# kakaoenterprise/JORLDY

Hardware: AMD Instinct MI355X
Metric: env_steps_per_s (PPO CartPole sync, W=8 workers/GPU, T=128) (higher is better)
Workload: dtype f32

## Files before the change

### jorldy_amd/csrc/jh_collect.hip

```cpp
#include <chrono>

#include "jh_common.h"

struct jh_persist;
int jh_persist_create(jh_pponet* n, jh_persist** out);
void jh_persist_destroy(jh_persist* p);
int jh_persist_begin(jh_persist* p, int W, int T, hipStream_t st, int split = 0);
unsigned jh_persist_publish(jh_persist* p, int W, const float* h_obs);
unsigned jh_persist_seq(const jh_persist* p);
void jh_persist_publish_rows(jh_persist* p, int r0, int r1, const float* h_obs, unsigned tag);
int jh_persist_collect_range(jh_persist* p, int r0, int n_rows, unsigned tag, float* h_heads);
int jh_persist_collect(jh_persist* p, int W, unsigned tag, float* h_heads);
int jh_persist_collect_rows(jh_persist* p, const int* rows, int n_rows, unsigned tag, float* h_heads);
void jh_persist_abort(jh_persist* p);
bool jh_persist_gave_up(const jh_persist* p);
void jh_persist_dump_debug(jh_persist* p, int T);

namespace {
struct Level {
  void* env = nullptr;
  int S = 0;
  std::vector<float> next, obs, rw;
  std::vector<uint8_t> dn;
  std::vector<int64_t> act;
  void init(int rows, int S_) {
    S = S_;
    next.resize((size_t)S * rows); obs.resize((size_t)S * rows); rw.resize(rows); dn.resize(rows); act.resize(rows);
    for (int i = 0; i < rows; ++i) act[i] = i & 1;
  }
};
inline int fork_step(const jh_env_vtbl& vt, Level& dst, const void* src, int n_src) {
  for (int i = 0; i < n_src; ++i) { vt.copy_row(dst.env, 2 * i, src, i); vt.copy_row(dst.env, 2 * i + 1, src, i); }
  int rc = vt.step(dst.env, 0, 2 * n_src, dst.act.data(), dst.next.data(), dst.rw.data(), dst.dn.data());
  if (rc) return rc;
  return vt.obs(dst.env, 0, 2 * n_src, dst.obs.data());
}
inline void copy_level_row(const jh_env_vtbl& vt, Level& d, int di, const Level& s_, int si) {
  vt.copy_row(d.env, di, s_.env, si);
  const size_t S = (size_t)d.S;
  memcpy(&d.next[S * (size_t)di], &s_.next[S * (size_t)si], sizeof(float) * S);
  memcpy(&d.obs[S * (size_t)di], &s_.obs[S * (size_t)si], sizeof(float) * S);
  d.rw[di] = s_.rw[si];
  d.dn[di] = s_.dn[si];
}
}

struct jh_collector {
  jh_ctx* ctx = nullptr;
  jh_pponet* net = nullptr;
  jh_env_vtbl vt{};
  void* env = nullptr;
  jh_store* store = nullptr;
  int W = 0, S = 0, A = 0;
  int no = 0;
  bool cont = false;
  int col_state = 0, col_action = 1, col_reward = 2, col_next = 3, col_done = 4;
  std::vector<float> obs, next_obs, reward, heads, act_f;
  std::vector<int64_t> act_i;
  std::vector<uint8_t> done;
  bool dbg = false, dbg_persist = false;
  double dbg_publish = 0.0, dbg_wait = 0.0;
  long dbg_n = 0;
  jh_persist* persist = nullptr;
  int mode = 1;
  int lookahead = 1;
  bool split = false;
  Level lv[4];
  void *spec = nullptr, *spec2 = nullptr, *spec3 = nullptr;
  float *cap_h0 = nullptr, *cap_h1 = nullptr, *cap_v = nullptr, *cap_nv = nullptr;
  int64_t cap_rows = 0;
  const void* ride_src[2] = {nullptr, nullptr};
  void* ride_dst[2] = {nullptr, nullptr};
  int64_t ride_bytes[2] = {0, 0};
  void* run = nullptr;
  unsigned *gate_h = nullptr, *gate_d = nullptr, gate_seq = 0;
  int prelaunched_T = 0;
  double t_act = 0, t_env = 0, t_total = 0;
  double t_first = 0, t_extra = 0, t_commit = 0;
  int64_t runs = 0;
  int64_t steps = 0;
};

struct RunState;
static void run_state_alloc(jh_collector* c);
static void run_state_free(jh_collector* c);

static int cart_obs(void* e, int32_t r0, int32_t r1, float* o);
static int ctl_obs(void* e, int32_t r0, int32_t r1, float* o);

static int collector_create(jh_ctx* ctx, jh_pponet* net, const jh_env_vtbl* vt, void* env, jh_store* store, const int32_t* cols,
                            jh_collector** out) {
  JH_ARG(ctx && net && vt && env && store && cols && out);
  JH_ARG(vt->obs && vt->step && vt->W > 0 && vt->S > 0 && vt->A > 0);
  const int W = vt->W, S = vt->S, A = vt->A;
  const bool cont = vt->continuous != 0;
  JH_ARG(net->S == S && net->A == A && (net->cont != 0) == cont);
  JH_ARG(W <= net->max_act_rows);
  for (int i = 0; i < 5; ++i) JH_ARG(cols[i] >= 0 && cols[i] < store->n_cols);
  JH_ARG(store->cols[cols[0]].dtype == JH_F32 && store->cols[cols[0]].elems == S);
  if (cont) JH_ARG(store->cols[cols[1]].dtype == JH_F32 && store->cols[cols[1]].elems == A);
  else JH_ARG(store->cols[cols[1]].dtype == JH_I64 && store->cols[cols[1]].elems == 1);
  JH_ARG(store->cols[cols[2]].dtype == JH_F32 && store->cols[cols[2]].elems == 1);
  JH_ARG(store->cols[cols[3]].dtype == JH_F32 && store->cols[cols[3]].elems == S);
  JH_ARG(store->cols[cols[4]].dtype == JH_U8 && store->cols[cols[4]].elems == 1);
  JH_HIP(hipSetDevice(ctx->device));
  jh_collector* c = new jh_collector();
  c->ctx = ctx; c->net = net; c->vt = *vt; c->env = env; c->store = store; c->W = W; c->S = S; c->A = A; c->cont = cont;
  c->col_state = cols[0]; c->col_action = cols[1]; c->col_reward = cols[2]; c->col_next = cols[3]; c->col_done = cols[4];
  c->no = (cont ? 2 * A : A) + 1;
  c->dbg = getenv("JH_COLLECT_DEBUG") != nullptr;
  c->dbg_persist = getenv("JH_PERSIST_DEBUG") != nullptr;
  if (const char* e = getenv("JH_COLLECT_PERSISTENT")) c->mode = atoi(e);
  if (c->mode == 1 && W <= 32 && W * S <= 512) {
    if (jh_persist_create(net, &c->persist) != JH_OK) c->persist = nullptr;
  }
  const bool forkable = vt->fork_alloc && vt->fork_free && vt->copy_row;
  if (c->persist && forkable && !cont && A == 2 && 3 * W <= 32 && 3 * W * S <= 128) {
    const char* e = getenv("JH_COLLECT_LOOKAHEAD");
    c->lookahead = e ? (atoi(e) >= 2 ? 2 : 1) : 2;
    if (c->lookahead == 2) {
      c->spec = vt->fork_alloc(env, 2 * W); c->spec2 = vt->fork_alloc(env, 4 * W); c->spec3 = vt->fork_alloc(env, 8 * W);
      if (!c->spec || !c->spec2 || !c->spec3) c->lookahead = 1;
    }
  }
  {
    const char* e = getenv("JH_COLLECT_SPLIT");
    c->split = c->persist && c->lookahead != 2 && W == 32 && (vt->obs == cart_obs || vt->obs == ctl_obs) && !(e && atoi(e) == 0);
  }
  c->obs.resize((size_t)S * W);
  c->next_obs.resize((size_t)S * W);
  c->act_i.resize(W);
  c->act_f.resize((size_t)A * W);
  c->reward.resize(W);
  c->done.resize(W);
  c->heads.resize((size_t)c->no * W);
  run_state_alloc(c);
  *out = c;
  return JH_OK;
}

static int cart_obs(void* e, int32_t r0, int32_t r1, float* o) { jh_cartpole_obs_rows((const jh_cartpole*)e, r0, r1, o); return JH_OK; }
static int cart_step(void* e, int32_t r0, int32_t r1, const void* a, float* nx, float* rw, uint8_t* dn) {
  jh_cartpole_step_rows((jh_cartpole*)e, r0, r1, (const int64_t*)a, nx, rw, dn);
  return JH_OK;
}
static void* cart_fork_alloc(void*, int32_t rows) {
  jh_cartpole* e = nullptr;
  return jh_cartpole_create(rows, 0, &e) == JH_OK ? e : nullptr;
}
static void cart_fork_free(void* e) { jh_cartpole_destroy((jh_cartpole*)e); }
static void cart_copy_row(void* d_, int32_t di, const void* s_, int32_t si) {
  jh_cartpole* d = (jh_cartpole*)d_;
  const jh_cartpole* s = (const jh_cartpole*)s_;
  memcpy(&d->s[4 * (size_t)di], &s->s[4 * (size_t)si], sizeof(double) * 4);
  d->t[di] = s->t[si];
  d->rng[di] = s->rng[si];
}
static int ctl_obs(void* e, int32_t r0, int32_t r1, float* o) {
  const jh_control* c = (const jh_control*)e;
  if (r0 < 0 || r1 > c->W || r0 >= r1) return jh_fail(JH_ERR_ARG, "jh_control: rows %d..%d of %d", r0, r1, c->W);
  jh_control_obs_rows(c, r0, r1, o);
  return JH_OK;
}
static int ctl_step(void* e, int32_t r0, int32_t r1, const void* a, float* nx, float* rw, uint8_t* dn) {
  jh_control* c = (jh_control*)e;
  if (r0 < 0 || r1 > c->W || r0 >= r1) return jh_fail(JH_ERR_ARG, "jh_control: rows %d..%d of %d", r0, r1, c->W);
  jh_control_step_rows(c, r0, r1, (const float*)a, nx, rw, dn);
  return JH_OK;
}

JH_EXPORT int jh_collector_create(jh_ctx* ctx, jh_pponet* net, jh_cartpole* env, jh_store* store,
                                  const int32_t* cols ,
                                  jh_collector** out) {
  JH_ARG(env != nullptr);
  const jh_env_vtbl vt{env->W, 4, 2, 0, cart_obs, cart_step, cart_fork_alloc, cart_fork_free, cart_copy_row};
  return collector_create(ctx, net, &vt, env, store, cols, out);
}

JH_EXPORT int jh_collector_create_control(jh_ctx* ctx, jh_pponet* net, jh_control* env, jh_store* store, const int32_t* cols,
                                          jh_collector** out) {
  JH_ARG(env != nullptr);
  const jh_env_vtbl vt{env->W, env->S, env->A, 1, ctl_obs, ctl_step, nullptr, nullptr, nullptr};
  return collector_create(ctx, net, &vt, env, store, cols, out);
}

JH_EXPORT int jh_collector_create_env(jh_ctx* ctx, jh_pponet* net, const jh_env_vtbl* vt, void* env, jh_store* store, const int32_t* cols,
                                      jh_collector** out) {
  return collector_create(ctx, net, vt, env, store, cols, out);
}

JH_EXPORT void jh_collector_destroy(jh_collector* c) {
  if (!c) return;
  if (c->persist) {
    (void)hipSetDevice(c->ctx->device);
    (void)hipDeviceSynchronize();
    jh_persist_destroy(c->persist);
  }
  if (c->gate_h) (void)hipHostFree(c->gate_h);
  if (c->spec) c->vt.fork_free(c->spec);
  if (c->spec2) c->vt.fork_free(c->spec2);
  if (c->spec3) c->vt.fork_free(c->spec3);
  run_state_free(c);
  delete c;
}

JH_EXPORT int jh_collector_set_capture(jh_collector* c, float* d_h0, float* d_h1, float* d_value, float* d_next_value, int64_t rows) {
  JH_ARG(c != nullptr);
  if (!d_value) { c->cap_h0 = c->cap_h1 = c->cap_v = c->cap_nv = nullptr; c->cap_rows = 0; return JH_OK; }
  JH_ARG(d_h0 && d_next_value && rows > 0 && (!c->cont || d_h1));
  c->cap_h0 = d_h0; c->cap_h1 = c->cont ? d_h1 : nullptr; c->cap_v = d_value; c->cap_nv = d_next_value; c->cap_rows = rows;
  return JH_OK;
}

JH_EXPORT int jh_collector_set_ride_along(jh_collector* c, int32_t slot, const void* d_src_mapped, void* d_dst, int64_t bytes) {
  JH_ARG(c != nullptr && slot >= 0 && slot < 2 && bytes >= 0 && (bytes == 0 || (d_src_mapped && d_dst)));
  c->ride_src[slot] = d_src_mapped; c->ride_dst[slot] = d_dst; c->ride_bytes[slot] = bytes;
  return JH_OK;
}

static int collector_steps(const jh_collector* c, int T) {
  const int extra = (c->cap_v && c->cap_rows == (int64_t)c->W * T) ? 1 : 0;
  return (c->lookahead == 2 ? (T + 1) / 2 : T) + extra;
}
static int collector_rows(const jh_collector* c) { return c->lookahead == 2 ? 3 * c->W : c->W; }

JH_EXPORT int jh_collector_prelaunch(jh_collector* c, int32_t T, jh_stream stream) {
  JH_ARG(c != nullptr && T > 0);
  if (!c->persist || c->prelaunched_T) return JH_OK;
  const int steps = collector_steps(c, T);
  int rc = jh_persist_begin(c->persist, collector_rows(c), steps, jh_s(stream), c->split);
  if (rc == JH_OK) c->prelaunched_T = steps;
  return rc;
}

struct RunState {
  bool active = false, cap = false, persistent = false, early = false;
  int T = 0, steps = 0;
  int64_t n = 0;
  float *st = nullptr, *ns = nullptr, *rw = nullptr;
  uint8_t* dn = nullptr;
  int64_t* ac_i = nullptr;
  float* ac_f = nullptr;
  jh_pinned_slab* cap_slab = nullptr;
  float *ch0 = nullptr, *ch1 = nullptr, *cv = nullptr, *cnv = nullptr;
  int stall_t = -1, stall_h = -1;
};
static RunState& run_state(jh_collector* c) { return *static_cast<RunState*>(c->run); }
static void run_state_alloc(jh_collector* c) { c->run = new RunState(); }
static void run_state_free(jh_collector* c) { delete static_cast<RunState*>(c->run); c->run = nullptr; }

static int run_commit(jh_collector* c, RunState& r, int rc_in, const unsigned* wait_flag, unsigned wait_val, hipStream_t st) {
  if (rc_in != JH_OK && wait_flag == nullptr) {
    (void)jh_store_stage_abort(c->store, st);
    if (r.cap_slab) (void)jh_ctx_slab_release(c->ctx, r.cap_slab, st);
    r.cap_slab = nullptr;
    for (int q = 0; q < 2; ++q) { c->ride_src[q] = nullptr; c->ride_dst[q] = nullptr; c->ride_bytes[q] = 0; }
    return rc_in;
  }
  const int A = c->A;
  const int64_t n = r.n;
  const void* xs[6]; void* xd[6]; int64_t xb[6]; int k = 0;
  if (r.cap && rc_in == JH_OK) {
    const char* dev0 = (const char*)r.cap_slab->dev;
    auto job = [&](const float* h, float* d, size_t floats) { xs[k] = dev0 + ((const char*)h - (const char*)r.cap_slab->host); xd[k] = d; xb[k] = (int64_t)(sizeof(float) * floats); ++k; };
    job(r.ch0, c->cap_h0, (size_t)n * A);
    if (c->cont) job(r.ch1, c->cap_h1, (size_t)n * A);
    job(r.cv, c->cap_v, (size_t)n);
    job(r.cnv, c->cap_nv, (size_t)n);
  }
  for (int q = 0; q < 2; ++q) {
    if (rc_in == JH_OK && c->ride_bytes[q] > 0) { xs[k] = c->ride_src[q]; xd[k] = c->ride_dst[q]; xb[k] = c->ride_bytes[q]; ++k; }
    c->ride_src[q] = nullptr; c->ride_dst[q] = nullptr; c->ride_bytes[q] = 0;
  }
  const int rc2 = jh_store_stage_commit_gated(c->store, k, xs, xd, xb, wait_flag, wait_val, st);
  if (r.cap_slab) (void)jh_ctx_slab_release(c->ctx, r.cap_slab, st);
  r.cap_slab = nullptr;
  return rc_in ? rc_in : rc2;
}

static int run_prepare(jh_collector* c, int T, hipStream_t st) {
  if (c->gate_h) {
    const unsigned lost = __atomic_load_n(c->gate_h + 1, __ATOMIC_ACQUIRE);
    if (lost) {
      __atomic_store_n(c->gate_h + 1, 0u, __ATOMIC_RELEASE);
      return jh_fail(JH_ERR_STATE, "the commit launch of an earlier run (tag %u) timed out waiting for its release: that rollout never reached the store and the "
                                   "learner behind it ran on stale rows -- the agent's weights are not trustworthy", lost);
    }
  }
  RunState& r = run_state(c);
  const int W = c->W, A = c->A;
  r = RunState();
  r.T = T;
  r.n = (int64_t)W * T;
  r.cap = c->cap_v && c->cap_rows == r.n;
  r.steps = collector_steps(c, T);
  if (const char* e = getenv("JH_COLLECT_TEST_STALL")) (void)sscanf(e, "%d,%d", &r.stall_t, &r.stall_h);
  void* cols[16] = {};
  int rc = jh_store_stage_begin(c->store, r.n, cols);
  if (rc) return rc;
  r.st = (float*)cols[c->col_state];
  r.ns = (float*)cols[c->col_next];
  r.rw = (float*)cols[c->col_reward];
  r.dn = (uint8_t*)cols[c->col_done];
  r.ac_i = (int64_t*)cols[c->col_action];
  r.ac_f = (float*)cols[c->col_action];
  if (r.cap) {
    const size_t fl = (size_t)r.n * A * (c->cont ? 2 : 1) + 2 * (size_t)r.n;
    rc = jh_ctx_slab(c->ctx, sizeof(float) * fl, &r.cap_slab);
    if (rc) { (void)jh_store_stage_commit(c->store, st); return rc; }
    r.ch0 = (float*)r.cap_slab->host;
    r.ch1 = c->cont ? r.ch0 + (size_t)r.n * A : nullptr;
    r.cv = r.ch0 + (size_t)r.n * A * (c->cont ? 2 : 1);
    r.cnv = r.cv + r.n;
  }
  r.persistent = c->persist != nullptr;
  if (r.persistent) {
    const int pre = c->prelaunched_T;
    c->prelaunched_T = 0;
    if (pre != r.steps || jh_persist_gave_up(c->persist)) {
      if (pre && !jh_persist_gave_up(c->persist)) {
        jh_persist_abort(c->persist);
        (void)hipStreamSynchronize(st);
      }
      rc = jh_persist_begin(c->persist, collector_rows(c), r.steps, st, c->split);
      if (rc) r.persistent = false;
    }
  }
  r.active = true;
  return JH_OK;
}

using Clock = std::chrono::steady_clock;
static double secs(Clock::time_point a, Clock::time_point b) { return std::chrono::duration<double>(b - a).count(); }

static void count_act(jh_collector* c, const RunState& r, int t, double dt) {
  c->t_act += dt;
  if (t == r.T) c->t_extra += dt;
  else if (t == 0) c->t_first += dt;
}

static const void* act_of(const jh_collector* c, int w) {
  return c->cont ? (const void*)(c->act_f.data() + (size_t)c->A * w) : (const void*)(c->act_i.data() + w);
}

static void sample_row(jh_collector* c, const float* z, int w, int training) {
  if (c->cont) jh_sample_continuous(c->net, z, w, training, c->act_f.data() + (size_t)w * c->A);
  else c->act_i[w] = jh_sample_discrete(c->net, z, w, training);
}

static void capture_row(const jh_collector* c, const RunState& r, int w, int t, const float* z) {
  if (!r.cap) return;
  const int A = c->A;
  const float v = z[c->no - 1];
  if (t > 0) r.cnv[(size_t)w * r.T + (t - 1)] = v;
  if (t == r.T) return;
  const size_t row = (size_t)w * r.T + t;
  r.cv[row] = v;
  memcpy(r.ch0 + row * A, z, sizeof(float) * A);
  if (c->cont) memcpy(r.ch1 + row * A, z + A, sizeof(float) * A);
}

static void store_row(const jh_collector* c, const RunState& r, int w, int t, const float* s, const float* s_next, const void* a, float rw, uint8_t dn) {
  const int S = c->S, A = c->A;
  const size_t row = (size_t)w * r.T + t;
  memcpy(r.st + S * row, s, sizeof(float) * S);
  memcpy(r.ns + S * row, s_next, sizeof(float) * S);
  if (c->cont) memcpy(r.ac_f + A * row, a, sizeof(float) * A);
  else r.ac_i[row] = *(const int64_t*)a;
  r.rw[row] = rw;
  r.dn[row] = dn;
}

static int step_rows(jh_collector* c, const RunState& r, int w0, int w1, int t) {
  const int rc = c->vt.step(c->env, w0, w1, act_of(c, 0), c->next_obs.data(), c->reward.data(), c->done.data());
  if (rc) return rc;
  const size_t S = (size_t)c->S;
  for (int w = w0; w < w1; ++w) store_row(c, r, w, t, &c->obs[S * w], &c->next_obs[S * w], act_of(c, w), c->reward[w], c->done[w]);
  return JH_OK;
}

static int act_launch(jh_collector* c, int r0, int n, int training, hipStream_t st) {
  const int A = c->A, no = c->no;
  std::vector<float> mu((size_t)n * A), ls((size_t)n * A), v(n);
  const float* obs = c->obs.data() + (size_t)r0 * c->S;
  const int rc = c->cont ? jh_pponet_act_continuous(c->net, n, obs, c->act_f.data() + (size_t)r0 * A, mu.data(), ls.data(), v.data(), training, (jh_stream)st)
                         : jh_pponet_act_discrete(c->net, n, obs, c->act_i.data() + r0, mu.data(), v.data(), training, (jh_stream)st);
  if (rc) return rc;
  for (int k = 0; k < n; ++k) {
    float* z = c->heads.data() + (size_t)(r0 + k) * no;
    memcpy(z, &mu[(size_t)k * A], sizeof(float) * A);
    if (c->cont) memcpy(z + A, &ls[(size_t)k * A], sizeof(float) * A);
    z[no - 1] = v[k];
  }
  return JH_OK;
}

static int env_failed(jh_collector* c, int rc) {
  jh_persist_abort(c->persist);
  return rc;
}

static int kernel_gave_up(jh_collector* c, const RunState& r, int t, hipStream_t st, int* t_done) {
  jh_persist_abort(c->persist);
  if (r.early)
    return jh_fail(JH_ERR_STATE, "the persistent acting kernel gave up at step %d of a run whose commit was enqueued ahead (jh_collector_begin): "
                                 "no observations for ~0.2 s; use jh_collector_run for environments that may stall", t);
  JH_HIP(hipStreamSynchronize(st));
  *t_done = t;
  return JH_OK;
}


static int run_loop_exchange(jh_collector* c, int training, hipStream_t st, int* t_done) {
  RunState& r = run_state(c);
  const int W = c->W, T = r.T, steps = T + (r.cap ? 1 : 0);
  for (int t = 0; t < steps; ++t) {
    const bool extra = t == T;
    int rc = c->vt.obs(c->env, 0, W, c->obs.data());
    if (rc) return env_failed(c, rc);
    const auto t0 = Clock::now();
    const unsigned tag = jh_persist_publish(c->persist, W, c->obs.data());
    const auto tp = c->dbg ? Clock::now() : t0;
    rc = jh_persist_collect(c->persist, W, tag, c->heads.data());
    if (c->dbg) {
      c->dbg_publish += secs(t0, tp);
      c->dbg_wait += secs(tp, Clock::now());
      c->dbg_n += 1;
    }
    if (rc) return kernel_gave_up(c, r, t, st, t_done);
    for (int w = 0; w < W; ++w) {
      const float* z = c->heads.data() + (size_t)w * c->no;
      if (!extra) sample_row(c, z, w, training);
      capture_row(c, r, w, t, z);
    }
    if (!extra) c->net->act_ctr += 1;
    const auto t1 = Clock::now();
    count_act(c, r, t, secs(t0, t1));
    if (extra) break;
    rc = step_rows(c, r, 0, W, t);
    if (rc) return env_failed(c, rc);
    c->t_env += secs(t1, Clock::now());
    c->steps += 1;
  }
  *t_done = steps;
  if (c->dbg_persist && (c->runs % 16) == 15) jh_persist_dump_debug(c->persist, T);
  if (c->dbg_n > 0 && (c->runs % 4) == 3) {
    fprintf(stderr, "[jh_collect] one timestep per exchange, per step: publish %.2f us, wait + read of the heads %.2f us (sampling + bookkeeping + env step: the rest of act / env)\n",
            c->dbg_publish / c->dbg_n * 1e6, c->dbg_wait / c->dbg_n * 1e6);
    c->dbg_publish = c->dbg_wait = 0.0;
    c->dbg_n = 0;
  }
  return JH_OK;
}

static int run_loop_split(jh_collector* c, int training, hipStream_t st, int* t_done) {
  RunState& r = run_state(c);
  const int W = c->W, T = r.T, steps = T + (r.cap ? 1 : 0), HR = 16;
  const unsigned base = jh_persist_seq(c->persist);
  bool dead = false;
  int rc = c->vt.obs(c->env, 0, W, c->obs.data());
  if (rc) return env_failed(c, rc);
  for (int h = 0; h < 2; ++h) jh_persist_publish_rows(c->persist, h * HR, (h + 1) * HR, c->obs.data(), base + 1);
  for (int t = 0; t < steps; ++t) {
    const bool extra = t == T;
    for (int h = 0; h < 2; ++h) {
      const int r0 = h * HR, r1 = r0 + HR;
      const auto t0 = Clock::now();
      if (t == r.stall_t && h == r.stall_h) {
        while (secs(t0, Clock::now()) < 0.35) {}
      }
      rc = jh_persist_collect_range(c->persist, r0, HR, base + (unsigned)t + 1, c->heads.data() + (size_t)r0 * c->no);
      if (rc) {
        rc = kernel_gave_up(c, r, t, st, t_done);
        if (rc || h == 0) return rc;
        const uint64_t ctr = c->net->act_ctr;
        rc = act_launch(c, r0, HR, 0, st);
        if (rc) return rc;
        c->net->act_ctr = ctr;
        dead = true;
      }
      for (int w = r0; w < r1; ++w) {
        const float* z = c->heads.data() + (size_t)w * c->no;
        if (!extra) sample_row(c, z, w, training);
        capture_row(c, r, w, t, z);
      }
      if (h == 1 && !extra) c->net->act_ctr += 1;
      const auto t1 = Clock::now();
      count_act(c, r, t, secs(t0, t1));
      if (extra) continue;
      rc = step_rows(c, r, r0, r1, t);
      if (rc) return env_failed(c, rc);
      if (t + 1 < steps && !dead) {
        rc = c->vt.obs(c->env, r0, r1, c->obs.data());
        if (rc) return env_failed(c, rc);
        jh_persist_publish_rows(c->persist, r0, r1, c->obs.data(), base + (unsigned)t + 2);
      }
      c->t_env += secs(t1, Clock::now());
    }
    if (!extra) c->steps += 1;
    if (dead) {
      *t_done = t + 1;
      return JH_OK;
    }
  }
  *t_done = steps;
  return JH_OK;
}

static int run_loop_lookahead(jh_collector* c, int training, hipStream_t st, int* t_done) {
  RunState& r = run_state(c);
  const int W = c->W, S = c->S, T = r.T, steps = T + (r.cap ? 1 : 0), no = c->no;
  void* e = c->env;
  const jh_env_vtbl& vt = c->vt;
  Level &L1 = c->lv[0], &L2 = c->lv[1], &L3 = c->lv[2], &tmp = c->lv[3];
  L1.env = c->spec; L2.env = c->spec2; L3.env = c->spec3;
  L1.init(2 * W, S); L2.init(4 * W, S); L3.init(8 * W, S);
  std::vector<float> pub((size_t)3 * W * S), pub_next((size_t)3 * W * S), hz((size_t)W * no), hz2((size_t)W * no);
  std::vector<int> pick(W);
  std::vector<int64_t> a0(W), a1(W);
  int t = 0;
  const bool dbg = c->dbg;
  double d_fork = 0, d_wait = 0, d_sample = 0, d_publish = 0, d_book = 0;
  int n_ex = 0;
  int rc = fork_step(vt, L1, e, W);
  if (!rc) rc = vt.obs(e, 0, W, pub.data());
  if (rc) return env_failed(c, rc);
  memcpy(pub.data() + (size_t)W * S, L1.obs.data(), sizeof(float) * (size_t)2 * W * S);
  auto t0 = Clock::now();
  unsigned tag = jh_persist_publish(c->persist, 3 * W, pub.data());
  while (t < steps) {
    const bool extra = t == T;
    const bool two = !extra && t + 1 < T;
    const int t_next = t + (two ? 2 : 1);
    const auto q0 = dbg ? Clock::now() : Clock::time_point();
    if (!extra) {
      rc = fork_step(vt, L2, L1.env, 2 * W);
      if (!rc && two && t_next < steps) rc = fork_step(vt, L3, L2.env, 4 * W);
      if (rc) return env_failed(c, rc);
    }
    const auto q1 = dbg ? Clock::now() : q0;
    rc = jh_persist_collect_rows(c->persist, nullptr, W, tag, hz.data());
    const auto q2 = dbg ? Clock::now() : q0;
    if (rc) return kernel_gave_up(c, r, t, st, t_done);
    if (!extra) {
      for (int w = 0; w < W; ++w) {
        a0[w] = jh_sample_discrete(c->net, hz.data() + (size_t)w * no, w, training);
        pick[w] = W + 2 * w + (int)a0[w];
      }
      c->net->act_ctr += 1;
      if (two) {
        rc = jh_persist_collect_rows(c->persist, pick.data(), W, tag, hz2.data());
        if (rc) return rc;
        for (int w = 0; w < W; ++w) a1[w] = jh_sample_discrete(c->net, hz2.data() + (size_t)w * no, w, training);
        c->net->act_ctr += 1;
      }
    }
    const auto t1 = Clock::now();
    if (dbg) { d_fork += secs(q0, q1); d_wait += secs(q1, q2); d_sample += secs(q2, t1); ++n_ex; }
    unsigned tag_next = 0;
    auto t0_next = t1;
    if (!extra && t_next < steps) {
      for (int w = 0; w < W; ++w) {
        const int k1 = 2 * w + (int)a0[w];
        if (two) {
          const int k2 = 2 * k1 + (int)a1[w];
          memcpy(&pub_next[(size_t)S * w], &L2.obs[(size_t)S * k2], sizeof(float) * S);
          memcpy(&pub_next[(size_t)S * (W + 2 * w)], &L3.obs[(size_t)S * 2 * k2], sizeof(float) * 2 * S);
        } else {
          memcpy(&pub_next[(size_t)S * w], &L1.obs[(size_t)S * k1], sizeof(float) * S);
          memcpy(&pub_next[(size_t)S * (W + 2 * w)], &L2.obs[(size_t)S * 2 * k1], sizeof(float) * 2 * S);
        }
      }
      t0_next = Clock::now();
      tag_next = jh_persist_publish(c->persist, 3 * W, pub_next.data());
    }
    const auto q3 = dbg ? Clock::now() : t1;
    if (dbg) d_publish += secs(t1, q3);
    for (int w = 0; w < W; ++w) {
      capture_row(c, r, w, t, hz.data() + (size_t)w * no);
      if (two) capture_row(c, r, w, t + 1, hz2.data() + (size_t)w * no);
    }
    count_act(c, r, t, secs(t0, t1));
    if (extra) {
      t = t_next;
      break;
    }
    if (!two) { tmp.env = L3.env; tmp.init(2 * W, S); }
    for (int w = 0; w < W; ++w) {
      const int k1 = 2 * w + (int)a0[w];
      store_row(c, r, w, t, &pub[(size_t)S * w], &L1.next[(size_t)S * k1], &a0[w], L1.rw[k1], L1.dn[k1]);
      if (two) {
        const int k2 = 2 * k1 + (int)a1[w];
        store_row(c, r, w, t + 1, &L1.obs[(size_t)S * k1], &L2.next[(size_t)S * k2], &a1[w], L2.rw[k2], L2.dn[k2]);
        vt.copy_row(e, w, L2.env, k2);
        if (t_next < steps) {
          copy_level_row(vt, L1, 2 * w, L3, 2 * k2);
          copy_level_row(vt, L1, 2 * w + 1, L3, 2 * k2 + 1);
        }
      } else {
        vt.copy_row(e, w, L1.env, k1);
        copy_level_row(vt, tmp, 2 * w, L2, 2 * k1);
        copy_level_row(vt, tmp, 2 * w + 1, L2, 2 * k1 + 1);
      }
    }
    if (!two)
      for (int i = 0; i < 2 * W; ++i) copy_level_row(vt, L1, i, tmp, i);
    c->steps += two ? 2 : 1;
    const auto t2 = Clock::now();
    if (dbg) d_book += secs(q3, t2);
    c->t_env += secs(t1, t2);
    t = t_next;
    tag = tag_next;
    t0 = t0_next;
    pub.swap(pub_next);
  }
  *t_done = t;
  if (dbg && n_ex > 0 && (c->runs % 16) == 15)
    fprintf(stderr, "[jh_collect] host us per exchange (%d exchanges): fork %.2f  wait %.2f  sample %.2f  publish %.2f  book %.2f\n", n_ex, d_fork / n_ex * 1e6,
            d_wait / n_ex * 1e6, d_sample / n_ex * 1e6, d_publish / n_ex * 1e6, d_book / n_ex * 1e6);
  if (c->dbg_persist && (c->runs % 16) == 15) jh_persist_dump_debug(c->persist, collector_steps(c, T));
  return JH_OK;
}

static int run_loop_per_launch(jh_collector* c, int training, hipStream_t st, int t_begin) {
  RunState& r = run_state(c);
  if (r.early) return jh_fail(JH_ERR_STATE, "jh_collector_begin needs the persistent acting kernel (W <= 32, W * S <= 512, JH_COLLECT_PERSISTENT != 0)");
  const int W = c->W, T = r.T, steps = T + (r.cap ? 1 : 0);
  for (int t = t_begin; t < steps; ++t) {
    const bool extra = t == T;
    int rc = c->vt.obs(c->env, 0, W, c->obs.data());
    if (rc) return rc;
    const auto t0 = Clock::now();
    rc = act_launch(c, 0, W, training, st);
    if (rc) return rc;
    if (extra) c->net->act_ctr -= 1;
    for (int w = 0; w < W; ++w) capture_row(c, r, w, t, c->heads.data() + (size_t)w * c->no);
    const auto t1 = Clock::now();
    count_act(c, r, t, secs(t0, t1));
    if (extra) break;
    rc = step_rows(c, r, 0, W, t);
    if (rc) return rc;
    c->t_env += secs(t1, Clock::now());
    c->steps += 1;
  }
  return JH_OK;
}

static int run_loop(jh_collector* c, int training, hipStream_t st) {
  RunState& r = run_state(c);
  int t = 0;
  if (r.persistent) {
    const int rc = c->lookahead == 2 ? run_loop_lookahead(c, training, st, &t)
                   : c->split        ? run_loop_split(c, training, st, &t)
                                     : run_loop_exchange(c, training, st, &t);
    if (rc) return rc;
  }
  return t < r.T + (r.cap ? 1 : 0) ? run_loop_per_launch(c, training, st, t) : JH_OK;
}

JH_EXPORT int jh_collector_run(jh_collector* c, int32_t T, int32_t training, jh_stream stream) {
  JH_ARG(c != nullptr && T > 0);
  if (run_state(c).active) return jh_fail(JH_ERR_STATE, "jh_collector_run inside a jh_collector_begin / jh_collector_loop pair");
  int rc = run_prepare(c, T, jh_s(stream));
  if (rc) return rc;
  rc = run_loop(c, training, jh_s(stream));
  const auto tc = std::chrono::steady_clock::now();
  rc = run_commit(c, run_state(c), rc, nullptr, 0, jh_s(stream));
  c->t_commit += std::chrono::duration<double>(std::chrono::steady_clock::now() - tc).count();
  c->runs += 1;
  run_state(c).active = false;
  return rc;
}

JH_EXPORT int jh_collector_begin(jh_collector* c, int32_t T, jh_stream stream) {
  JH_ARG(c != nullptr && T > 0);
  if (run_state(c).active) return jh_fail(JH_ERR_STATE, "jh_collector_begin twice without jh_collector_loop");
  if (!c->persist) return jh_fail(JH_ERR_STATE, "jh_collector_begin needs the persistent acting kernel (W <= 32, W * S <= 512, JH_COLLECT_PERSISTENT != 0)");
  if (!c->gate_h) {
    JH_HIP(hipHostMalloc((void**)&c->gate_h, 64, hipHostMallocMapped));
    JH_HIP(hipHostGetDevicePointer((void**)&c->gate_d, c->gate_h, 0));
    c->gate_h[0] = 0;
    c->gate_h[1] = 0;
  }
  int rc = run_prepare(c, T, jh_s(stream));
  if (rc) return rc;
  RunState& r = run_state(c);
  if (!r.persistent || !jh_store_commit_is_one_launch(c->store, r.n)) {
    r.early = false;
    return JH_OK;
  }
  r.early = true;
  c->gate_seq = (c->gate_seq + 1) & 0x7fffffffu;
  if (c->gate_seq == 0) c->gate_seq = 1;
  const auto tc = std::chrono::steady_clock::now();
  rc = run_commit(c, r, JH_OK, c->gate_d, c->gate_seq, jh_s(stream));
  c->t_commit += std::chrono::duration<double>(std::chrono::steady_clock::now() - tc).count();
  if (rc) {
    __atomic_store_n(c->gate_h, c->gate_seq, __ATOMIC_RELEASE);
    r.active = false;
  }
  return rc;
}

JH_EXPORT int jh_collector_loop(jh_collector* c, int32_t training, jh_stream stream) {
  JH_ARG(c != nullptr);
  RunState& r = run_state(c);
  if (!r.active) return jh_fail(JH_ERR_STATE, "jh_collector_loop without jh_collector_begin");
  int rc = run_loop(c, training, jh_s(stream));
  if (r.early) {
    __atomic_store_n(c->gate_h, rc == JH_OK ? c->gate_seq : (c->gate_seq | 0x80000000u), __ATOMIC_RELEASE);
  } else {
    const auto tc = std::chrono::steady_clock::now();
    rc = run_commit(c, r, rc, nullptr, 0, jh_s(stream));
    c->t_commit += std::chrono::duration<double>(std::chrono::steady_clock::now() - tc).count();
  }
  c->runs += 1;
  r.active = false;
  return rc;
}

JH_EXPORT int jh_collector_stats_detail(jh_collector* c, double* out6) {
  JH_ARG(c && out6);
  const double r = c->runs > 0 ? (double)c->runs : 1.0;
  out6[0] = c->t_first / r * 1e6;
  out6[1] = c->t_extra / r * 1e6;
  out6[2] = c->t_commit / r * 1e6;
  const double inner = (double)c->steps - (double)c->runs;
  out6[3] = inner > 0 ? (c->t_act - c->t_first - c->t_extra) / inner * 1e6 : 0.0;
  out6[4] = (double)c->runs;
  out6[5] = (double)c->steps;
  return JH_OK;
}

JH_EXPORT int jh_collector_stats(jh_collector* c, double* act_us_per_step, double* env_us_per_step, int32_t reset) {
  JH_ARG(c != nullptr);
  const double n = c->steps > 0 ? (double)c->steps : 1.0;
  if (act_us_per_step) *act_us_per_step = c->t_act / n * 1e6;
  if (env_us_per_step) *env_us_per_step = c->t_env / n * 1e6;
  if (reset) { c->t_act = c->t_env = c->t_first = c->t_extra = c->t_commit = 0; c->steps = 0; c->runs = 0; }
  return JH_OK;
}
```

### jorldy_amd/csrc/jh_persist.hip

```cpp
#if defined(__x86_64__)
#include <emmintrin.h>
#endif

#include "jh_common.h"

typedef float f32x4 __attribute__((ext_vector_type(4)));

struct PersistArgs {
  int W, S, H, n_out, T, G;
  const float *W1, *b1, *W2, *b2;
  const float* wh[12];
  const float* hbias[12];
  const unsigned long long* obs_gran;
  float4* part;
  int rows_ld;
  unsigned* abort_flag;
  unsigned seq0;
  long max_polls;
  unsigned long long* dbg;
  int period;
  unsigned long long* mbox;
  float4* dpart;
  int split;
};

__device__ __forceinline__ void persist_poll_issue(const void* gsrc, unsigned lds_off) {
  unsigned keep;
  asm volatile("s_mov_b32 %0, m0\n\ts_mov_b32 m0, %2\n\ts_nop 0\n\tglobal_load_lds_dwordx4 %1, off sc0 sc1\n\ts_mov_b32 m0, %0"
               : "=&s"(keep) : "v"(gsrc), "s"(lds_off) : "memory");
}

template <int SP, int NCH, int D, int PI>
__global__ void __launch_bounds__(256, 1) jh_act_persist_kernel(PersistArgs p) {
  constexpr bool W1LDS = SP > 8;
  constexpr int NJ = 2 * PI;
  __shared__ __attribute__((aligned(16))) unsigned long long s_ring[D][128 * PI];
  __shared__ __attribute__((aligned(16))) float s_w1[W1LDS ? 64 * NCH * SP : 4];
  __shared__ __attribute__((aligned(16))) float s_x[2][16][SP];
  __shared__ __attribute__((aligned(16))) float s_acc[2][4][64][4];
  __shared__ float s_h2[16][17];
  __shared__ float s_wh[12][16];
  __shared__ float s_b2[16], s_hb[12];
  __shared__ __attribute__((aligned(16))) float s_out[16][12];
  __shared__ int s_go[2];
  __shared__ __attribute__((aligned(16))) f32x4 s_red[32][64];
  const int H = p.H, S = p.S;
  const int lane = threadIdx.x & 63, wid = __builtin_amdgcn_readfirstlane(threadIdx.x >> 6);
  const int tiles_n = H / 16;
  const int tile = blockIdx.x % tiles_n, rt = blockIdx.x / tiles_n, n0 = tile * 16;
  const int r = lane & 15, kq = lane >> 4;
  const int kbeg = wid * 16 * NCH;
  float w2f[NCH][4], b1f[NCH][4], w1f[NCH][4][W1LDS ? 1 : SP];
#pragma unroll
  for (int u = 0; u < NCH; ++u) {
    const int kb = kbeg + 16 * u + 4 * kq;
#pragma unroll
    for (int j = 0; j < 4; ++j) {
      w2f[u][j] = p.W2[(size_t)(n0 + r) * H + kb + j];
      b1f[u][j] = p.b1[kb + j];
      if (!W1LDS) {
#pragma unroll
        for (int q = 0; q < SP; ++q) w1f[u][j][q] = q < S ? p.W1[(size_t)(kb + j) * S + q] : 0.f;
      }
    }
  }
  if (W1LDS) {
    for (int i = threadIdx.x; i < H * SP; i += 256) {
      const int k = i / SP, q = i - k * SP;
      s_w1[i] = q < S ? p.W1[(size_t)k * S + q] : 0.f;
    }
  }
  for (int i = threadIdx.x; i < 12 * 16; i += 256) {
    const int o = i >> 4, c = i & 15;
    s_wh[o][c] = o < p.n_out ? p.wh[o][n0 + c] : 0.f;
  }
  if (threadIdx.x < 16) s_b2[threadIdx.x] = p.b2[n0 + threadIdx.x];
  if (threadIdx.x < 12) s_hb[threadIdx.x] = threadIdx.x < p.n_out ? *p.hbias[threadIdx.x] : 0.f;
  for (int i = threadIdx.x; i < 2 * 16 * SP; i += 256) (&s_x[0][0][0])[i] = 0.f;
  for (int i = threadIdx.x; i < D * 128 * PI; i += 256) (&s_ring[0][0])[i] = 0ull;
  __syncthreads();

  const int g0 = p.split ? rt * 16 * S : 0;
  const int n_gran = p.split ? (p.W - 16 * rt < 16 ? p.W - 16 * rt : 16) * S : p.W * S;
  const int n16 = (n_gran + 1) >> 1;
  const char* my_src = reinterpret_cast<const char*>(p.obs_gran + g0) + 16 * (lane < n16 ? lane : 0);
  const bool poller = !p.mbox || (p.split ? tile == 0 : blockIdx.x == 0);
  unsigned long long next_issue = 0;
  int slot = 0;
  const unsigned ring_lane = (unsigned)(uintptr_t)&s_ring[0][0] + 8u * (unsigned)lane;
  __builtin_amdgcn_s_waitcnt(0x0F70);
  if (wid == 0 && poller) {
#pragma unroll
    for (int d = 0; d < D; ++d) {
#pragma unroll
      for (int q = 0; q < PI; ++q)
        if (64 * q + lane < n16) persist_poll_issue(my_src + 1024 * q, __builtin_amdgcn_readfirstlane((unsigned)(uintptr_t)&s_ring[d][0]) + 1024u * q);
    }
    next_issue = wall_clock64();
  }

  for (int t = 1; t <= p.T; ++t) {
    const int par = t & 1;
    const unsigned tag = p.seq0 + (unsigned)t;
    if (wid == 0 && !poller) {
      bool ok = false;
      for (long spin = 0; spin < p.max_polls * 4; ++spin) {
        unsigned long long gq[NJ];
        bool mine = true;
#pragma unroll
        for (int j = 0; j < NJ; ++j) {
          const int g = 64 * j + lane;
          gq[j] = (j == 0 || 64 * j < n_gran) ? __hip_atomic_load(p.mbox + g0 + (g < n_gran ? g : 0), __ATOMIC_RELAXED, __HIP_MEMORY_SCOPE_AGENT) : 0ull;
          mine = mine && (g >= n_gran || (unsigned)(gq[j] >> 32) == tag);
        }
        if (__all(mine)) {
#pragma unroll
          for (int j = 0; j < NJ; ++j) {
            const int g = 64 * j + lane, gg = g0 + g;
            if (g < n_gran && (gg / S) >> 4 == rt) s_x[par][(gg / S) & 15][gg % S] = __uint_as_float((unsigned)gq[j]);
          }
          ok = true;
          break;
        }
        if ((spin & 1023) == 1023 && __hip_atomic_load(p.abort_flag, __ATOMIC_RELAXED, __HIP_MEMORY_SCOPE_SYSTEM) != 0) break;
      }
      if (lane == 0) s_go[par] = ok ? 1 : 0;
    } else if (wid == 0) {
      bool ok = false;
      for (long spin = 0; spin < p.max_polls; ++spin) {
        asm volatile("s_waitcnt vmcnt(%0)" ::"n"(PI * (D - 1)) : "memory");
        unsigned long long gq[NJ];
        {
          const unsigned ra = ring_lane + (unsigned)slot * (1024u * PI);
          if constexpr (PI == 1) {
            asm volatile("ds_read_b64 %0, %2\n\tds_read_b64 %1, %2 offset:512\n\ts_waitcnt lgkmcnt(0)" : "=&v"(gq[0]), "=&v"(gq[1]) : "v"(ra) : "memory");
          } else if constexpr (PI == 2) {
            asm volatile("ds_read_b64 %0, %4\n\tds_read_b64 %1, %4 offset:512\n\tds_read_b64 %2, %4 offset:1024\n\tds_read_b64 %3, %4 offset:1536\n\ts_waitcnt lgkmcnt(0)"
                         : "=&v"(gq[0]), "=&v"(gq[1]), "=&v"(gq[2]), "=&v"(gq[3]) : "v"(ra) : "memory");
          } else if constexpr (PI == 3) {
            asm volatile("ds_read_b64 %0, %6\n\tds_read_b64 %1, %6 offset:512\n\tds_read_b64 %2, %6 offset:1024\n\tds_read_b64 %3, %6 offset:1536\n\t"
                         "ds_read_b64 %4, %6 offset:2048\n\tds_read_b64 %5, %6 offset:2560\n\ts_waitcnt lgkmcnt(0)"
                         : "=&v"(gq[0]), "=&v"(gq[1]), "=&v"(gq[2]), "=&v"(gq[3]), "=&v"(gq[4]), "=&v"(gq[5]) : "v"(ra) : "memory");
          } else {
            static_assert(PI == 4, "1 .. 4 poll instructions per poll are spelled out");
            asm volatile("ds_read_b64 %0, %8\n\tds_read_b64 %1, %8 offset:512\n\tds_read_b64 %2, %8 offset:1024\n\tds_read_b64 %3, %8 offset:1536\n\t"
                         "ds_read_b64 %4, %8 offset:2048\n\tds_read_b64 %5, %8 offset:2560\n\tds_read_b64 %6, %8 offset:3072\n\tds_read_b64 %7, %8 offset:3584\n\ts_waitcnt lgkmcnt(0)"
                         : "=&v"(gq[0]), "=&v"(gq[1]), "=&v"(gq[2]), "=&v"(gq[3]), "=&v"(gq[4]), "=&v"(gq[5]), "=&v"(gq[6]), "=&v"(gq[7]) : "v"(ra) : "memory");
          }
        }
        bool mine = true;
#pragma unroll
        for (int j = 0; j < NJ; ++j) mine = mine && (64 * j + lane >= n_gran || (unsigned)(gq[j] >> 32) == tag);
        const bool done = __all(mine);
        if (done) {
#pragma unroll
          for (int j = 0; j < NJ; ++j) {
            const int g = 64 * j + lane, gg = g0 + g;
            if (g < n_gran) {
              if ((gg / S) >> 4 == rt) s_x[par][(gg / S) & 15][gg % S] = __uint_as_float((unsigned)gq[j]);
              if (p.mbox) __hip_atomic_store(p.mbox + gg, gq[j], __ATOMIC_RELAXED, __HIP_MEMORY_SCOPE_AGENT);
            }
          }
        }
        if (p.period > 0 && !done) {
          while (wall_clock64() < next_issue) __builtin_amdgcn_s_sleep(1);
        }
        next_issue = wall_clock64() + (unsigned long long)p.period;
#pragma unroll
        for (int q = 0; q < PI; ++q)
          if (64 * q + lane < n16) persist_poll_issue(my_src + 1024 * q, __builtin_amdgcn_readfirstlane((unsigned)(uintptr_t)&s_ring[slot][0]) + 1024u * q);
        slot = __builtin_amdgcn_readfirstlane(slot + 1 == D ? 0 : slot + 1);
        if (done) { ok = true; break; }
        if ((spin & 255) == 255 && __hip_atomic_load(p.abort_flag, __ATOMIC_RELAXED, __HIP_MEMORY_SCOPE_SYSTEM) != 0) break;
      }
      if (lane == 0) s_go[par] = ok ? 1 : 0;
    }
    __syncthreads();
    if (p.dbg && blockIdx.x == 0 && threadIdx.x == 0) { p.dbg[(t - 1) * 8 + 0] = wall_clock64(); p.dbg[(t - 1) * 8 + 1] = __builtin_readcyclecounter(); }
    if (!s_go[par]) {
      if (threadIdx.x == 0) __hip_atomic_store(p.abort_flag, 2u, __ATOMIC_RELAXED, __HIP_MEMORY_SCOPE_SYSTEM);
      break;
    }
    float xr[SP];
#pragma unroll
    for (int q4 = 0; q4 < SP / 4; ++q4) {
      const float4 v = *reinterpret_cast<const float4*>(&s_x[par][r][4 * q4]);
      xr[4 * q4] = v.x; xr[4 * q4 + 1] = v.y; xr[4 * q4 + 2] = v.z; xr[4 * q4 + 3] = v.w;
    }
    f32x4 acc = (f32x4){0.f, 0.f, 0.f, 0.f}, acc2 = (f32x4){0.f, 0.f, 0.f, 0.f};
#pragma unroll
    for (int u = 0; u < NCH; ++u) {
#pragma unroll
      for (int j = 0; j < 4; ++j) {
        float a = 0.f;
        if (W1LDS) {
          const float* wr = s_w1 + (size_t)(kbeg + 16 * u + 4 * kq + j) * SP;
#pragma unroll
          for (int q4 = 0; q4 < SP / 4; ++q4) {
            const float4 w = *reinterpret_cast<const float4*>(wr + 4 * q4);
            a = fmaf(xr[4 * q4], w.x, a); a = fmaf(xr[4 * q4 + 1], w.y, a); a = fmaf(xr[4 * q4 + 2], w.z, a); a = fmaf(xr[4 * q4 + 3], w.w, a);
          }
        } else {
#pragma unroll
          for (int q = 0; q < SP; ++q) a = fmaf(xr[q], w1f[u][j][q], a);
        }
        a += b1f[u][j];
        a = a > 0.f ? a : 0.f;
        if (j & 1) acc2 = __builtin_amdgcn_mfma_f32_16x16x4f32(a, w2f[u][j], acc2, 0, 0, 0);
        else acc = __builtin_amdgcn_mfma_f32_16x16x4f32(a, w2f[u][j], acc, 0, 0, 0);
      }
    }
#pragma unroll
    for (int i = 0; i < 4; ++i) s_acc[par][wid][lane][i] = acc[i] + acc2[i];
    __syncthreads();
    if (wid == 0) {
      float hv[4];
#pragma unroll
      for (int i = 0; i < 4; ++i) {
        float v = ((s_acc[par][0][lane][i] + s_acc[par][1][lane][i]) + s_acc[par][2][lane][i]) + s_acc[par][3][lane][i];
        v += s_b2[r];
        hv[i] = v > 0.f ? v : 0.f;
      }
#pragma unroll
      for (int i = 0; i < 4; ++i) s_h2[kq * 4 + i][r] = hv[i];
      __builtin_amdgcn_wave_barrier();
      __builtin_amdgcn_fence(__ATOMIC_RELEASE, "workgroup");
      f32x4 ph = (f32x4){0.f, 0.f, 0.f, 0.f};
#pragma unroll
      for (int c = 0; c < 4; ++c) {
        const float av = s_h2[r][4 * c + kq];
        const float bv = r < 12 ? s_wh[r][4 * c + kq] : 0.f;
        ph = __builtin_amdgcn_mfma_f32_16x16x4f32(av, bv, ph, 0, 0, 0);
      }
      if (r < 12) {
#pragma unroll
        for (int i = 0; i < 4; ++i) s_out[kq * 4 + i][r] = ph[i] + (tile == 0 ? s_hb[r] : 0.f);
      }
      __builtin_amdgcn_wave_barrier();
      __builtin_amdgcn_fence(__ATOMIC_RELEASE, "workgroup");
      const int g = lane >> 4, row = lane & 15;
      if (g < p.G && 16 * rt + row < p.W) {
        const f32x4 gq = (f32x4){s_out[row][3 * g], s_out[row][3 * g + 1], s_out[row][3 * g + 2], __uint_as_float(tag)};
        if (p.dpart) {
          float4* dst = p.dpart + ((size_t)(rt * p.G + g) * 16 + row) * tiles_n + tile;
          asm volatile("global_store_dwordx4 %0, %1, off sc1\n\ts_nop 1" ::"v"(dst), "v"(gq) : "memory");
        } else {
          float4* dst = p.part + ((size_t)tile * p.G + g) * p.rows_ld + 16 * rt + row;
          asm volatile("global_store_dwordx4 %0, %1, off sc0 sc1\n\ts_nop 1" ::"v"(dst), "v"(gq) : "memory");
        }
      }
    }
    if (p.dpart && tile == 0) {
      const int g = lane >> 4, row = lane & 15;
      const bool mine = g < p.G && 16 * rt + row < p.W;
      const int per = tiles_n / 4;
      bool ok = true;
      if (mine) {
        const float4* src = p.dpart + ((size_t)(rt * p.G + g) * 16 + row) * tiles_n + wid * per;
        f32x4 q[8];
        long spin = 0;
        for (;;) {
          const float4* a1 = per > 4 ? src + 4 : src;
          asm volatile("global_load_dwordx4 %0, %8, off sc1\n\tglobal_load_dwordx4 %1, %9, off sc1\n\tglobal_load_dwordx4 %2, %10, off sc1\n\t"
                       "global_load_dwordx4 %3, %11, off sc1\n\tglobal_load_dwordx4 %4, %12, off sc1\n\tglobal_load_dwordx4 %5, %12, off offset:16 sc1\n\t"
                       "global_load_dwordx4 %6, %12, off offset:32 sc1\n\tglobal_load_dwordx4 %7, %12, off offset:48 sc1\n\ts_waitcnt vmcnt(0)"
                       : "=&v"(q[0]), "=&v"(q[1]), "=&v"(q[2]), "=&v"(q[3]), "=&v"(q[4]), "=&v"(q[5]), "=&v"(q[6]), "=&v"(q[7])
                       : "v"(src), "v"(src + (per > 1 ? 1 : 0)), "v"(src + (per > 2 ? 2 : 0)), "v"(src + (per > 2 ? 3 : 0)), "v"(a1)
                       : "memory");
          bool all = true, newer = false;
#pragma unroll
          for (int j = 0; j < 8; ++j) {
            const unsigned seen = __float_as_uint(q[j][3]);
            if (j < per) {
              all = all && seen == tag;
              newer = newer || (int)(seen - tag) > 0;
            }
          }
          if (all) break;
          if (newer || ++spin > 2000000L || ((spin & 1023) == 1023 && __hip_atomic_load(p.abort_flag, __ATOMIC_RELAXED, __HIP_MEMORY_SCOPE_SYSTEM) != 0)) { ok = false; break; }
        }
#pragma unroll
        for (int j = 0; j < 8; ++j)
          if (j < per) s_red[wid * per + j][lane] = ok ? q[j] : (f32x4){0.f, 0.f, 0.f, __uint_as_float(tag + 0x40000000u)};
      }
      __syncthreads();
      if (wid == 1 && mine) {
        float z0 = 0.f, z1 = 0.f, z2 = 0.f;
        bool good = true;
        for (int tt = 0; tt < tiles_n; ++tt) {
          const f32x4 v = s_red[tt][lane];
          good = good && __float_as_uint(v[3]) == tag;
          z0 += v[0]; z1 += v[1]; z2 += v[2];
        }
        if (good) {
          const f32x4 gq = (f32x4){z0, z1, z2, __uint_as_float(tag)};
          float4* dst = p.part + (size_t)g * p.rows_ld + 16 * rt + row;
          asm volatile("global_store_dwordx4 %0, %1, off sc0 sc1\n\ts_nop 1" ::"v"(dst), "v"(gq) : "memory");
        }
      }
    }
    if (p.dbg && blockIdx.x == 0 && threadIdx.x == 0) { p.dbg[(t - 1) * 8 + 4] = wall_clock64(); p.dbg[(t - 1) * 8 + 5] = __builtin_readcyclecounter(); }
  }
  asm volatile("s_waitcnt vmcnt(0)" ::: "memory");
}

constexpr int kPersistMaxGranules = 512;
struct jh_persist {
  jh_pponet* net = nullptr;
  unsigned long long* gran_h = nullptr;
  unsigned long long* gran_d = nullptr;
  float4 *part_h = nullptr, *part_d = nullptr;
  unsigned *flag_h = nullptr, *flag_d = nullptr;
  unsigned seq = 0;
  int tiles = 0, n_out = 0, G = 0;
  int rows_ld = 16;
  unsigned long long *dbg_h = nullptr, *dbg_d = nullptr;
  unsigned long long* mbox = nullptr;
  float4* dpart = nullptr;
  bool reduced = false;
  int rows_published = 0;
  bool split = false;
};

static int persist_heads(const jh_pponet* n) { return (n->cont ? 2 * n->A : n->A) + 1; }

int jh_persist_create(jh_pponet* n, jh_persist** out) {
  JH_ARG(n && out);
  const int H = n->H, S = n->S;
  JH_ARG(S >= 1 && S <= 16 && (H == 64 || H == 128 || H == 256 || H == 512) && persist_heads(n) <= 12);
  jh_persist* p = new jh_persist();
  p->net = n;
  p->tiles = H / 16;
  p->n_out = persist_heads(n);
  p->G = (p->n_out + 2) / 3;
  JH_HIP(hipHostMalloc((void**)&p->gran_h, sizeof(unsigned long long) * kPersistMaxGranules, hipHostMallocMapped));
  JH_HIP(hipHostGetDevicePointer((void**)&p->gran_d, p->gran_h, 0));
  const size_t part_bytes = sizeof(float4) * 32 * (size_t)p->tiles * p->G;
  JH_HIP(hipHostMalloc((void**)&p->part_h, part_bytes, hipHostMallocMapped));
  memset(p->part_h, 0, part_bytes);
  JH_HIP(hipHostGetDevicePointer((void**)&p->part_d, p->part_h, 0));
  JH_HIP(hipHostMalloc((void**)&p->flag_h, sizeof(unsigned) * 16, hipHostMallocMapped));
  JH_HIP(hipHostGetDevicePointer((void**)&p->flag_d, p->flag_h, 0));
  JH_HIP(hipMalloc((void**)&p->mbox, sizeof(unsigned long long) * kPersistMaxGranules));
  JH_HIP(hipMemset(p->mbox, 0, sizeof(unsigned long long) * kPersistMaxGranules));
  JH_HIP(hipMalloc((void**)&p->dpart, sizeof(float4) * (2 * 4 * 16 * (size_t)p->tiles + 8)));
  JH_HIP(hipMemset(p->dpart, 0, sizeof(float4) * (2 * 4 * 16 * (size_t)p->tiles + 8)));
  memset(p->gran_h, 0, sizeof(unsigned long long) * kPersistMaxGranules);
  memset(p->flag_h, 0, sizeof(unsigned) * 16);
  if (getenv("JH_PERSIST_DEBUG")) {
    p->dbg_h = (unsigned long long*)malloc(sizeof(unsigned long long) * 8 * 4096);
    JH_HIP(hipMalloc((void**)&p->dbg_d, sizeof(unsigned long long) * 8 * 4096));
  }
  p->seq = 1000;
  *out = p;
  return JH_OK;
}

void jh_persist_destroy(jh_persist* p) {
  if (!p) return;
  (void)hipHostFree(p->gran_h);
  (void)hipHostFree(p->part_h);
  (void)hipHostFree(p->flag_h);
  (void)hipFree(p->mbox);
  (void)hipFree(p->dpart);
  if (p->dbg_d) (void)hipFree(p->dbg_d);
  free(p->dbg_h);
  delete p;
}

template <int SP, int NCH>
static void persist_launch(int depth, int pi, int grid, hipStream_t st, const PersistArgs& a) {
  if (pi == 2) JH_LAUNCH_NAMED("jh_act_persist_kernel", (jh_act_persist_kernel<SP, NCH, 4, 2>), dim3(grid), dim3(256), 0, st, a);
  else if (pi == 3) JH_LAUNCH_NAMED("jh_act_persist_kernel", (jh_act_persist_kernel<SP, NCH, 4, 3>), dim3(grid), dim3(256), 0, st, a);
  else if (pi == 4) JH_LAUNCH_NAMED("jh_act_persist_kernel", (jh_act_persist_kernel<SP, NCH, 4, 4>), dim3(grid), dim3(256), 0, st, a);
  else if (depth >= 4) JH_LAUNCH_NAMED("jh_act_persist_kernel", (jh_act_persist_kernel<SP, NCH, 4, 1>), dim3(grid), dim3(256), 0, st, a);
  else if (depth >= 2) JH_LAUNCH_NAMED("jh_act_persist_kernel", (jh_act_persist_kernel<SP, NCH, 2, 1>), dim3(grid), dim3(256), 0, st, a);
  else JH_LAUNCH_NAMED("jh_act_persist_kernel", (jh_act_persist_kernel<SP, NCH, 1, 1>), dim3(grid), dim3(256), 0, st, a);
}

int jh_persist_begin(jh_persist* p, int W, int T, hipStream_t st, int split) {
  jh_pponet* n = p->net;
  JH_ARG(W > 0 && W <= 32 && W * n->S <= kPersistMaxGranules && T > 0 && (!split || W == 32));
  const int win = split ? 16 * n->S : W * n->S;
  const int pi = ((win + 1) / 2 + 63) / 64;
  PersistArgs a{};
  a.W = W; a.S = n->S; a.H = n->H; a.T = T; a.G = p->G;
  a.W1 = n->params + n->o_w1; a.b1 = n->params + n->o_b1; a.W2 = n->params + n->o_w2; a.b2 = n->params + n->o_b2;
  int o = 0;
  for (int k = 0; k < n->A; ++k, ++o) { a.wh[o] = n->params + n->o_wh0 + (int64_t)k * n->H; a.hbias[o] = n->params + n->o_bh0 + k; }
  if (n->cont)
    for (int k = 0; k < n->A; ++k, ++o) { a.wh[o] = n->params + n->o_wh1 + (int64_t)k * n->H; a.hbias[o] = n->params + n->o_bh1 + k; }
  a.wh[o] = n->params + n->o_wv; a.hbias[o] = n->params + n->o_bv; ++o;
  a.n_out = o;
  a.obs_gran = p->gran_d; a.part = p->part_d; a.abort_flag = p->flag_d;
  a.seq0 = p->seq;
  a.dbg = p->dbg_d;
  static const int depth = getenv("JH_PERSIST_DEPTH") ? atoi(getenv("JH_PERSIST_DEPTH")) : 4;
  static const int period = getenv("JH_PERSIST_PERIOD") ? atoi(getenv("JH_PERSIST_PERIOD")) : 10;
  a.period = depth > 1 ? period : 0;
  static const int relay = getenv("JH_PERSIST_RELAY") ? atoi(getenv("JH_PERSIST_RELAY")) : 1;
  a.mbox = relay ? p->mbox : nullptr;
  const int reduce = getenv("JH_PERSIST_REDUCE") ? atoi(getenv("JH_PERSIST_REDUCE")) : (split ? 1 : 0);
  p->reduced = reduce == 1;
  a.dpart = p->reduced ? p->dpart : nullptr;
  a.split = split ? 1 : 0;
  p->split = split != 0;
  a.max_polls = 600000;
  p->flag_h[0] = 0;
  const int nch = n->H / 64;
  const int sp = (n->S + 3) / 4 * 4;
  const int rt = W > 16 ? 2 : 1;
  p->rows_ld = 16 * rt;
  a.rows_ld = p->rows_ld;
  const int grid = p->tiles * rt;
#define JH_PERSIST_CASE(NCH)                                   \
  if (nch == NCH) {                                            \
    if (sp == 4) persist_launch<4, NCH>(depth, pi, grid, st, a);   \
    else if (sp == 8) persist_launch<8, NCH>(depth, pi, grid, st, a);   \
    else if (sp == 12) persist_launch<12, NCH>(depth, pi, grid, st, a); \
    else persist_launch<16, NCH>(depth, pi, grid, st, a);          \
  }
  JH_PERSIST_CASE(1) else JH_PERSIST_CASE(2) else JH_PERSIST_CASE(4) else JH_PERSIST_CASE(8)
#undef JH_PERSIST_CASE
  JH_LAUNCH_CHECK();
  return JH_OK;
}

unsigned jh_persist_publish(jh_persist* p, int W, const float* h_obs) {
  const unsigned tag = ++p->seq;
  p->rows_published = W;
  const int n = W * p->net->S;
  for (int i = 0; i < n; ++i) {
    unsigned bits;
    memcpy(&bits, h_obs + i, 4);
    __atomic_store_n(p->gran_h + i, ((unsigned long long)tag << 32) | bits, __ATOMIC_RELEASE);
  }
  return tag;
}

unsigned jh_persist_seq(const jh_persist* p) { return p->seq; }
void jh_persist_publish_rows(jh_persist* p, int r0, int r1, const float* h_obs, unsigned tag) {
  const int S = p->net->S;
  if (r1 > p->rows_published) p->rows_published = r1;
  for (int i = r0 * S; i < r1 * S; ++i) {
    unsigned bits;
    memcpy(&bits, h_obs + i, 4);
    __atomic_store_n(p->gran_h + i, ((unsigned long long)tag << 32) | bits, __ATOMIC_RELEASE);
  }
  if ((int)(tag - p->seq) > 0) p->seq = tag;
}

static int persist_collect(jh_persist* p, const int* rows, int n_rows, unsigned tag, float* h_heads, int r_first, bool block_order);
int jh_persist_collect_rows(jh_persist* p, const int* rows, int n_rows, unsigned tag, float* h_heads) {
  return persist_collect(p, rows, n_rows, tag, h_heads, 0, !rows && n_rows > 16);
}
int jh_persist_collect_range(jh_persist* p, int r0, int n_rows, unsigned tag, float* h_heads) { return persist_collect(p, nullptr, n_rows, tag, h_heads, r0, true); }
static int persist_collect(jh_persist* p, const int* rows, int n_rows, unsigned tag, float* h_heads, int r_first, bool block_order) {
  const int n_out = p->n_out, G = p->G, ld = p->rows_ld, tiles = p->reduced ? 1 : p->tiles;
  volatile unsigned* abort_w = p->flag_h;
  struct alignas(16) Gran16 { unsigned w[4]; };
  const Gran16* part = reinterpret_cast<const Gran16*>(p->part_h);
  float z[32][12];
  unsigned char have[32];
  JH_ARG(n_rows <= 32);
  if (block_order) {
    for (int k = 0; k < n_rows; ++k)
      for (int o = 0; o < 12; ++o) z[k][o] = 0.f;
    long spins = 0;
    for (int t = 0; t < tiles; ++t)
      for (int g = 0; g < G; ++g) {
        const Gran16* blk = part + ((size_t)t * G + g) * ld + r_first;
        for (;;) {
          bool all = true;
          for (int k = 0; k < n_rows; ++k)
            if (__atomic_load_n(reinterpret_cast<const unsigned*>(blk + k) + 3, __ATOMIC_ACQUIRE) != tag) { all = false; break; }
          if (all) break;
          if (++spins >= 40000000L || ((spins & 1023) == 1023 && *abort_w == 2u))
            return jh_fail(JH_ERR_STATE, "persistent acting kernel did not answer step tag %u", tag);
          __builtin_ia32_pause();
        }
        for (int k = 0; k < n_rows; ++k) {
          alignas(16) unsigned w4[4];
#if defined(__x86_64__)
          _mm_store_si128(reinterpret_cast<__m128i*>(w4), _mm_load_si128(reinterpret_cast<const __m128i*>(blk + k)));
#else
          memcpy(w4, blk + k, 16);
#endif
          if (w4[3] != tag) return jh_fail(JH_ERR_STATE, "persistent acting kernel: granule of step tag %u rewritten while it was read", tag);
          float f3[3];
          memcpy(f3, w4, 12);
          z[k][3 * g] += f3[0]; z[k][3 * g + 1] += f3[1]; z[k][3 * g + 2] += f3[2];
        }
      }
    for (int k = 0; k < n_rows; ++k) memcpy(h_heads + (size_t)k * n_out, z[k], sizeof(float) * n_out);
    return JH_OK;
  }
  int missing = n_rows;
  const int pf_rows = (!rows && p->rows_published > n_rows) ? p->rows_published - n_rows : 0;
  for (int k = 0; k < n_rows; ++k) have[k] = 0;
  for (long spin = 0; spin < 40000000L && missing; ++spin) {
    for (int k = 0; k < n_rows; ++k) {
      if (have[k]) continue;
      const int wq = rows ? rows[k] : k;
      float acc[12] = {0, 0, 0, 0, 0, 0, 0, 0, 0, 0, 0, 0};
      bool ok = true;
      for (int t = 0; t < tiles && ok; ++t)
        for (int g = 0; g < G; ++g) {
          const Gran16* gp = part + ((size_t)t * G + g) * ld + wq;
          if (__atomic_load_n(reinterpret_cast<const unsigned*>(gp) + 3, __ATOMIC_ACQUIRE) != tag) { ok = false; break; }
#if defined(__x86_64__)
          if (pf_rows > 0 && k == 0) {
            const char* q = reinterpret_cast<const char*>(part + ((size_t)t * G + g) * ld + n_rows);
            for (int b = 0; b < pf_rows * 16; b += 64) _mm_prefetch(q + b, _MM_HINT_T0);
          }
#endif
          alignas(16) unsigned w4[4];
#if defined(__x86_64__)
          _mm_store_si128(reinterpret_cast<__m128i*>(w4), _mm_load_si128(reinterpret_cast<const __m128i*>(gp)));
#else
          memcpy(w4, gp, 16);
#endif
          if (w4[3] != tag) { ok = false; break; }
          float f3[3];
          memcpy(f3, w4, 12);
          acc[3 * g] += f3[0]; acc[3 * g + 1] += f3[1]; acc[3 * g + 2] += f3[2];
        }
      if (ok) {
        memcpy(z[k], acc, sizeof(acc));
        have[k] = 1;
        --missing;
      }
    }
    if (missing) {
      if ((spin & 1023) == 1023 && *abort_w == 2u) break;
      __builtin_ia32_pause();
    }
  }
  if (missing) return jh_fail(JH_ERR_STATE, "persistent acting kernel did not answer step tag %u", tag);
  for (int k = 0; k < n_rows; ++k) memcpy(h_heads + (size_t)k * n_out, z[k], sizeof(float) * n_out);
  return JH_OK;
}

int jh_persist_collect(jh_persist* p, int W, unsigned tag, float* h_heads) { return jh_persist_collect_rows(p, nullptr, W, tag, h_heads); }

int jh_persist_heads(const jh_persist* p) { return p->n_out; }

void jh_persist_dump_debug(jh_persist* p, int T) {
  if (!p->dbg_h) return;
  (void)hipDeviceSynchronize();
  (void)hipMemcpy(p->dbg_h, p->dbg_d, sizeof(unsigned long long) * 8 * (size_t)T, hipMemcpyDeviceToHost);
  double a = 0, c = 0, cyc = 0;
  for (int t = 1; t < T; ++t) {
    const unsigned long long* d = p->dbg_h + (size_t)t * 8;
    const unsigned long long* pr = p->dbg_h + (size_t)(t - 1) * 8;
    a += (double)(d[0] - pr[4]);
    c += (double)(d[4] - d[0]);
    cyc += (double)(d[5] - d[1]) / ((double)(d[4] - d[0]) + 1e-9);
  }
  const double n = T - 1;
  fprintf(stderr, "[jh_persist] per step (wall_clock64 ticks = 10 ns): wait %.1f  compute %.1f ; shader clock ~%.0f MHz\n",
          a / n, c / n, cyc / n * 100.0);
}

bool jh_persist_gave_up(const jh_persist* p) { return __atomic_load_n(p->flag_h, __ATOMIC_ACQUIRE) == 2u; }

void jh_persist_abort(jh_persist* p) { __atomic_store_n(p->flag_h, 1u, __ATOMIC_RELEASE); }
```

Baseline: 1.220 million.

## Split lookahead exchange into two pipelined halves with variable row counts

```diff
diff --git a/jorldy_amd/csrc/jh_collect.hip b/jorldy_amd/csrc/jh_collect.hip
--- a/jorldy_amd/csrc/jh_collect.hip
+++ b/jorldy_amd/csrc/jh_collect.hip
@@ -5,11 +5,12 @@
 struct jh_persist;
 int jh_persist_create(jh_pponet* n, jh_persist** out);
 void jh_persist_destroy(jh_persist* p);
-int jh_persist_begin(jh_persist* p, int W, int T, hipStream_t st, int split = 0);
+bool jh_persist_can_split(const jh_persist* p, int rows0, int rows1);
+int jh_persist_begin(jh_persist* p, int W, int T, hipStream_t st, const int* half_rows);
 unsigned jh_persist_publish(jh_persist* p, int W, const float* h_obs);
 unsigned jh_persist_seq(const jh_persist* p);
-void jh_persist_publish_rows(jh_persist* p, int r0, int r1, const float* h_obs, unsigned tag);
-int jh_persist_collect_range(jh_persist* p, int r0, int n_rows, unsigned tag, float* h_heads);
+void jh_persist_publish_rows(jh_persist* p, int row0, int n, const float* h_obs, unsigned tag);
+int jh_persist_collect_range(jh_persist* p, int r0, int n_rows, unsigned tag, float* h_heads, int pf_rows);
 int jh_persist_collect(jh_persist* p, int W, unsigned tag, float* h_heads);
 int jh_persist_collect_rows(jh_persist* p, const int* rows, int n_rows, unsigned tag, float* h_heads);
 void jh_persist_abort(jh_persist* p);
@@ -29,11 +30,12 @@
     for (int i = 0; i < rows; ++i) act[i] = i & 1;
   }
 };
-inline int fork_step(const jh_env_vtbl& vt, Level& dst, const void* src, int n_src) {
-  for (int i = 0; i < n_src; ++i) { vt.copy_row(dst.env, 2 * i, src, i); vt.copy_row(dst.env, 2 * i + 1, src, i); }
-  int rc = vt.step(dst.env, 0, 2 * n_src, dst.act.data(), dst.next.data(), dst.rw.data(), dst.dn.data());
+inline int fork_step(const jh_env_vtbl& vt, Level& dst, const void* src, int i0, int i1) {
+  for (int i = i0; i < i1; ++i) { vt.copy_row(dst.env, 2 * i, src, i); vt.copy_row(dst.env, 2 * i + 1, src, i); }
+  const size_t r0 = 2 * (size_t)i0, S = (size_t)dst.S;
+  int rc = vt.step(dst.env, 2 * i0, 2 * i1, dst.act.data() + r0, dst.next.data() + S * r0, dst.rw.data() + r0, dst.dn.data() + r0);
   if (rc) return rc;
-  return vt.obs(dst.env, 0, 2 * n_src, dst.obs.data());
+  return vt.obs(dst.env, 2 * i0, 2 * i1, dst.obs.data() + S * r0);
 }
 inline void copy_level_row(const jh_env_vtbl& vt, Level& d, int di, const Level& s_, int si) {
   vt.copy_row(d.env, di, s_.env, si);
@@ -65,6 +67,7 @@
   int mode = 1;
   int lookahead = 1;
   bool split = false;
+  int w0[3] = {0, 0, 0};
   Level lv[4];
   void *spec = nullptr, *spec2 = nullptr, *spec3 = nullptr;
   float *cap_h0 = nullptr, *cap_h1 = nullptr, *cap_v = nullptr, *cap_nv = nullptr;
@@ -125,7 +128,11 @@
   }
   {
     const char* e = getenv("JH_COLLECT_SPLIT");
-    c->split = c->persist && c->lookahead != 2 && W == 32 && (vt->obs == cart_obs || vt->obs == ctl_obs) && !(e && atoi(e) == 0);
+    c->w0[1] = (W + 1) / 2;
+    c->w0[2] = W;
+    const int per_env = c->lookahead == 2 ? 3 : 1;
+    c->split = c->persist && W >= 2 && (c->lookahead == 2 || vt->obs == cart_obs || vt->obs == ctl_obs) && !(e && atoi(e) == 0) &&
+               jh_persist_can_split(c->persist, per_env * c->w0[1], per_env * (W - c->w0[1]));
   }
   c->obs.resize((size_t)S * W);
   c->next_obs.resize((size_t)S * W);
@@ -139,9 +146,9 @@
   return JH_OK;
 }
 
-static int cart_obs(void* e, int32_t r0, int32_t r1, float* o) { jh_cartpole_obs_rows((const jh_cartpole*)e, r0, r1, o); return JH_OK; }
+static int cart_obs(void* e, int32_t r0, int32_t r1, float* o) { jh_cartpole_obs_rows((const jh_cartpole*)e, r0, r1, o - 4 * (ptrdiff_t)r0); return JH_OK; }
 static int cart_step(void* e, int32_t r0, int32_t r1, const void* a, float* nx, float* rw, uint8_t* dn) {
-  jh_cartpole_step_rows((jh_cartpole*)e, r0, r1, (const int64_t*)a, nx, rw, dn);
+  jh_cartpole_step_rows((jh_cartpole*)e, r0, r1, (const int64_t*)a - r0, nx - 4 * (ptrdiff_t)r0, rw - r0, dn - r0);
   return JH_OK;
 }
 static void* cart_fork_alloc(void*, int32_t rows) {
@@ -159,13 +166,13 @@
 static int ctl_obs(void* e, int32_t r0, int32_t r1, float* o) {
   const jh_control* c = (const jh_control*)e;
   if (r0 < 0 || r1 > c->W || r0 >= r1) return jh_fail(JH_ERR_ARG, "jh_control: rows %d..%d of %d", r0, r1, c->W);
-  jh_control_obs_rows(c, r0, r1, o);
+  jh_control_obs_rows(c, r0, r1, o - (ptrdiff_t)c->S * r0);
   return JH_OK;
 }
 static int ctl_step(void* e, int32_t r0, int32_t r1, const void* a, float* nx, float* rw, uint8_t* dn) {
   jh_control* c = (jh_control*)e;
   if (r0 < 0 || r1 > c->W || r0 >= r1) return jh_fail(JH_ERR_ARG, "jh_control: rows %d..%d of %d", r0, r1, c->W);
-  jh_control_step_rows(c, r0, r1, (const float*)a, nx, rw, dn);
+  jh_control_step_rows(c, r0, r1, (const float*)a - (ptrdiff_t)c->A * r0, nx - (ptrdiff_t)c->S * r0, rw - r0, dn - r0);
   return JH_OK;
 }
 
@@ -223,12 +230,17 @@
   return (c->lookahead == 2 ? (T + 1) / 2 : T) + extra;
 }
 static int collector_rows(const jh_collector* c) { return c->lookahead == 2 ? 3 * c->W : c->W; }
+static int half_rows(const jh_collector* c, int h) { return (c->lookahead == 2 ? 3 : 1) * (c->w0[h + 1] - c->w0[h]); }
+static int collector_begin_kernel(jh_collector* c, int steps, hipStream_t st) {
+  const int hr[2] = {half_rows(c, 0), half_rows(c, 1)};
+  return jh_persist_begin(c->persist, collector_rows(c), steps, st, c->split ? hr : nullptr);
+}
 
 JH_EXPORT int jh_collector_prelaunch(jh_collector* c, int32_t T, jh_stream stream) {
   JH_ARG(c != nullptr && T > 0);
   if (!c->persist || c->prelaunched_T) return JH_OK;
   const int steps = collector_steps(c, T);
-  int rc = jh_persist_begin(c->persist, collector_rows(c), steps, jh_s(stream), c->split);
+  int rc = collector_begin_kernel(c, steps, jh_s(stream));
   if (rc == JH_OK) c->prelaunched_T = steps;
   return rc;
 }
@@ -322,7 +334,7 @@
         jh_persist_abort(c->persist);
         (void)hipStreamSynchronize(st);
       }
-      rc = jh_persist_begin(c->persist, collector_rows(c), r.steps, st, c->split);
+      rc = collector_begin_kernel(c, r.steps, st);
       if (rc) r.persistent = false;
     }
   }
@@ -372,9 +384,9 @@
 }
 
 static int step_rows(jh_collector* c, const RunState& r, int w0, int w1, int t) {
-  const int rc = c->vt.step(c->env, w0, w1, act_of(c, 0), c->next_obs.data(), c->reward.data(), c->done.data());
+  const size_t S = (size_t)c->S;
+  const int rc = c->vt.step(c->env, w0, w1, act_of(c, w0), c->next_obs.data() + S * w0, c->reward.data() + w0, c->done.data() + w0);
   if (rc) return rc;
-  const size_t S = (size_t)c->S;
   for (int w = w0; w < w1; ++w) store_row(c, r, w, t, &c->obs[S * w], &c->next_obs[S * w], act_of(c, w), c->reward[w], c->done[w]);
   return JH_OK;
 }
@@ -455,26 +467,26 @@
 
 static int run_loop_split(jh_collector* c, int training, hipStream_t st, int* t_done) {
   RunState& r = run_state(c);
-  const int W = c->W, T = r.T, steps = T + (r.cap ? 1 : 0), HR = 16;
+  const int W = c->W, S = c->S, T = r.T, steps = T + (r.cap ? 1 : 0);
   const unsigned base = jh_persist_seq(c->persist);
   bool dead = false;
   int rc = c->vt.obs(c->env, 0, W, c->obs.data());
   if (rc) return env_failed(c, rc);
-  for (int h = 0; h < 2; ++h) jh_persist_publish_rows(c->persist, h * HR, (h + 1) * HR, c->obs.data(), base + 1);
+  for (int h = 0; h < 2; ++h) jh_persist_publish_rows(c->persist, 16 * h, c->w0[h + 1] - c->w0[h], c->obs.data() + (size_t)S * c->w0[h], base + 1);
   for (int t = 0; t < steps; ++t) {
     const bool extra = t == T;
     for (int h = 0; h < 2; ++h) {
-      const int r0 = h * HR, r1 = r0 + HR;
+      const int r0 = c->w0[h], r1 = c->w0[h + 1];
       const auto t0 = Clock::now();
       if (t == r.stall_t && h == r.stall_h) {
         while (secs(t0, Clock::now()) < 0.35) {}
       }
-      rc = jh_persist_collect_range(c->persist, r0, HR, base + (unsigned)t + 1, c->heads.data() + (size_t)r0 * c->no);
+      rc = jh_persist_collect_range(c->persist, 16 * h, r1 - r0, base + (unsigned)t + 1, c->heads.data() + (size_t)r0 * c->no, 0);
       if (rc) {
         rc = kernel_gave_up(c, r, t, st, t_done);
         if (rc || h == 0) return rc;
         const uint64_t ctr = c->net->act_ctr;
-        rc = act_launch(c, r0, HR, 0, st);
+        rc = act_launch(c, r0, r1 - r0, 0, st);
         if (rc) return rc;
         c->net->act_ctr = ctr;
         dead = true;
@@ -491,9 +503,9 @@
       rc = step_rows(c, r, r0, r1, t);
       if (rc) return env_failed(c, rc);
       if (t + 1 < steps && !dead) {
-        rc = c->vt.obs(c->env, r0, r1, c->obs.data());
+        rc = c->vt.obs(c->env, r0, r1, c->obs.data() + (size_t)S * r0);
         if (rc) return env_failed(c, rc);
-        jh_persist_publish_rows(c->persist, r0, r1, c->obs.data(), base + (unsigned)t + 2);
+        jh_persist_publish_rows(c->persist, 16 * h, r1 - r0, c->obs.data() + (size_t)S * r0, base + (unsigned)t + 2);
       }
       c->t_env += secs(t1, Clock::now());
     }
@@ -510,115 +522,172 @@
 static int run_loop_lookahead(jh_collector* c, int training, hipStream_t st, int* t_done) {
   RunState& r = run_state(c);
   const int W = c->W, S = c->S, T = r.T, steps = T + (r.cap ? 1 : 0), no = c->no;
+  const int NP = c->split ? 2 : 1;
   void* e = c->env;
   const jh_env_vtbl& vt = c->vt;
   Level &L1 = c->lv[0], &L2 = c->lv[1], &L3 = c->lv[2], &tmp = c->lv[3];
   L1.env = c->spec; L2.env = c->spec2; L3.env = c->spec3;
   L1.init(2 * W, S); L2.init(4 * W, S); L3.init(8 * W, S);
-  std::vector<float> pub((size_t)3 * W * S), pub_next((size_t)3 * W * S), hz((size_t)W * no), hz2((size_t)W * no);
+  std::vector<float> pub_a((size_t)3 * W * S), pub_b((size_t)3 * W * S), hz((size_t)W * no), hz2((size_t)W * no);
   std::vector<int> pick(W);
   std::vector<int64_t> a0(W), a1(W);
-  int t = 0;
+  int e0s[2] = {0, 0}, e1s[2] = {W, W};
+  float *pub[2], *pub_next[2];
+  Clock::time_point t0[2];
+  for (int h = 0; h < NP; ++h) {
+    if (NP == 2) { e0s[h] = c->w0[h]; e1s[h] = c->w0[h + 1]; }
+    pub[h] = pub_a.data() + (size_t)3 * S * e0s[h];
+    pub_next[h] = pub_b.data() + (size_t)3 * S * e0s[h];
+  }
+  const unsigned base = jh_persist_seq(c->persist);
+  uint64_t ctr = c->net->act_ctr;
+  int t = 0, k = 0;
+  bool dead = false;
   const bool dbg = c->dbg;
   double d_fork = 0, d_wait = 0, d_sample = 0, d_publish = 0, d_book = 0;
   int n_ex = 0;
-  int rc = fork_step(vt, L1, e, W);
-  if (!rc) rc = vt.obs(e, 0, W, pub.data());
+  auto speculate = [&](int h, int t_at) -> int {
+    if (t_at == T) return JH_OK;
+    const bool two = t_at + 1 < T;
+    const auto q0 = dbg ? Clock::now() : Clock::time_point();
+    int rc = fork_step(vt, L2, L1.env, 2 * e0s[h], 2 * e1s[h]);
+    if (!rc && two && t_at + 2 < steps) rc = fork_step(vt, L3, L2.env, 4 * e0s[h], 4 * e1s[h]);
+    if (dbg) d_fork += secs(q0, Clock::now());
+    return rc;
+  };
+  auto heads_by_launch = [&](int h, auto x, float* out) -> int {
+    const int n = e1s[h] - e0s[h];
+    for (int i = 0; i < n; ++i) memcpy(&c->obs[(size_t)S * (e0s[h] + i)], x(i), sizeof(float) * S);
+    const uint64_t keep = c->net->act_ctr;
+    const int rc = act_launch(c, e0s[h], n, 0, st);
+    c->net->act_ctr = keep;
+    if (!rc) memcpy(out, c->heads.data() + (size_t)e0s[h] * no, sizeof(float) * (size_t)n * no);
+    return rc;
+  };
+  int rc = fork_step(vt, L1, e, 0, W);
+  if (!rc) rc = vt.obs(e, 0, W, c->obs.data());
   if (rc) return env_failed(c, rc);
-  memcpy(pub.data() + (size_t)W * S, L1.obs.data(), sizeof(float) * (size_t)2 * W * S);
-  auto t0 = Clock::now();
-  unsigned tag = jh_persist_publish(c->persist, 3 * W, pub.data());
+  for (int h = 0; h < NP; ++h) {
+    const int n = e1s[h] - e0s[h];
+    memcpy(pub[h], &c->obs[(size_t)S * e0s[h]], sizeof(float) * (size_t)n * S);
+    memcpy(pub[h] + (size_t)n * S, &L1.obs[(size_t)S * 2 * e0s[h]], sizeof(float) * (size_t)2 * n * S);
+    t0[h] = Clock::now();
+    jh_persist_publish_rows(c->persist, 16 * h, 3 * n, pub[h], base + 1);
+  }
+  auto last_t1 = t0[0];
+  for (int h = 0; h < NP; ++h) {
+    rc = speculate(h, 0);
+    if (rc) return env_failed(c, rc);
+  }
   while (t < steps) {
     const bool extra = t == T;
     const bool two = !extra && t + 1 < T;
     const int t_next = t + (two ? 2 : 1);
-    const auto q0 = dbg ? Clock::now() : Clock::time_point();
-    if (!extra) {
-      rc = fork_step(vt, L2, L1.env, 2 * W);
-      if (!rc && two && t_next < steps) rc = fork_step(vt, L3, L2.env, 4 * W);
-      if (rc) return env_failed(c, rc);
-    }
-    const auto q1 = dbg ? Clock::now() : q0;
-    rc = jh_persist_collect_rows(c->persist, nullptr, W, tag, hz.data());
-    const auto q2 = dbg ? Clock::now() : q0;
-    if (rc) return kernel_gave_up(c, r, t, st, t_done);
-    if (!extra) {
-      for (int w = 0; w < W; ++w) {
-        a0[w] = jh_sample_discrete(c->net, hz.data() + (size_t)w * no, w, training);
-        pick[w] = W + 2 * w + (int)a0[w];
-      }
-      c->net->act_ctr += 1;
-      if (two) {
-        rc = jh_persist_collect_rows(c->persist, pick.data(), W, tag, hz2.data());
+    const unsigned tag = base + (unsigned)k + 1;
+    for (int h = 0; h < NP; ++h) {
+      const int w0 = e0s[h], w1 = e1s[h], n = w1 - w0, rb = 16 * h;
+      const float* roots = pub[h];
+      if (t == r.stall_t && h == r.stall_h) {
+        const auto s0 = Clock::now();
+        while (secs(s0, Clock::now()) < 0.35) {}
+      }
+      const auto q1 = dbg ? Clock::now() : Clock::time_point();
+      c->net->act_ctr = ctr;
+      rc = jh_persist_collect_range(c->persist, rb, n, tag, hz.data() + (size_t)w0 * no, 2 * n);
+      const auto q2 = dbg ? Clock::now() : q1;
+      if (rc) {
+        rc = kernel_gave_up(c, r, t, st, t_done);
+        if (rc || h == 0) return rc;
+        dead = true;
+        rc = heads_by_launch(h, [&](int i) { return roots + (size_t)S * i; }, hz.data() + (size_t)w0 * no);
         if (rc) return rc;
-        for (int w = 0; w < W; ++w) a1[w] = jh_sample_discrete(c->net, hz2.data() + (size_t)w * no, w, training);
-        c->net->act_ctr += 1;
-      }
-    }
-    const auto t1 = Clock::now();
-    if (dbg) { d_fork += secs(q0, q1); d_wait += secs(q1, q2); d_sample += secs(q2, t1); ++n_ex; }
-    unsigned tag_next = 0;
-    auto t0_next = t1;
-    if (!extra && t_next < steps) {
-      for (int w = 0; w < W; ++w) {
+      }
+      if (!extra) {
+        for (int w = w0; w < w1; ++w) {
+          a0[w] = jh_sample_discrete(c->net, hz.data() + (size_t)w * no, w, training);
+          pick[w] = rb + n + 2 * (w - w0) + (int)a0[w];
+        }
+        if (two) {
+          c->net->act_ctr = ctr + 1;
+          rc = dead ? heads_by_launch(h, [&](int i) { return &L1.obs[(size_t)S * (2 * (w0 + i) + (int)a0[w0 + i])]; }, hz2.data() + (size_t)w0 * no)
+                    : jh_persist_collect_rows(c->persist, pick.data() + w0, n, tag, hz2.data() + (size_t)w0 * no);
+          if (rc) return rc;
+          for (int w = w0; w < w1; ++w) a1[w] = jh_sample_discrete(c->net, hz2.data() + (size_t)w * no, w, training);
+        }
+      }
+      const auto t1 = Clock::now();
+      if (dbg) { d_wait += secs(q1, q2); d_sample += secs(q2, t1); ++n_ex; }
+      auto t0_next = t1;
+      if (!extra && t_next < steps && !dead) {
+        float* pn = pub_next[h];
+        for (int w = w0; w < w1; ++w) {
+          const int i = w - w0, k1 = 2 * w + (int)a0[w];
+          if (two) {
+            const int k2 = 2 * k1 + (int)a1[w];
+            memcpy(&pn[(size_t)S * i], &L2.obs[(size_t)S * k2], sizeof(float) * S);
+            memcpy(&pn[(size_t)S * (n + 2 * i)], &L3.obs[(size_t)S * 2 * k2], sizeof(float) * 2 * S);
+          } else {
+            memcpy(&pn[(size_t)S * i], &L1.obs[(size_t)S * k1], sizeof(float) * S);
+            memcpy(&pn[(size_t)S * (n + 2 * i)], &L2.obs[(size_t)S * 2 * k1], sizeof(float) * 2 * S);
+          }
+        }
+        t0_next = Clock::now();
+        jh_persist_publish_rows(c->persist, rb, 3 * n, pn, tag + 1);
+      }
+      const auto q3 = dbg ? Clock::now() : t1;
+      if (dbg) d_publish += secs(t1, q3);
+      for (int w = w0; w < w1; ++w) {
+        capture_row(c, r, w, t, hz.data() + (size_t)w * no);
+        if (two) capture_row(c, r, w, t + 1, hz2.data() + (size_t)w * no);
+      }
+      count_act(c, r, t, secs(t0[h] > last_t1 ? t0[h] : last_t1, t1));
+      last_t1 = t1;
+      if (extra) continue;
+      const bool on = t_next < steps && !dead;
+      if (!two) { tmp.env = L3.env; tmp.init(2 * W, S); }
+      for (int w = w0; w < w1; ++w) {
         const int k1 = 2 * w + (int)a0[w];
+        store_row(c, r, w, t, roots + (size_t)S * (w - w0), &L1.next[(size_t)S * k1], &a0[w], L1.rw[k1], L1.dn[k1]);
         if (two) {
           const int k2 = 2 * k1 + (int)a1[w];
-          memcpy(&pub_next[(size_t)S * w], &L2.obs[(size_t)S * k2], sizeof(float) * S);
-          memcpy(&pub_next[(size_t)S * (W + 2 * w)], &L3.obs[(size_t)S * 2 * k2], sizeof(float) * 2 * S);
+          store_row(c, r, w, t + 1, &L1.obs[(size_t)S * k1], &L2.next[(size_t)S * k2], &a1[w], L2.rw[k2], L2.dn[k2]);
+          vt.copy_row(e, w, L2.env, k2);
+          if (on) {
+            copy_level_row(vt, L1, 2 * w, L3, 2 * k2);
+            copy_level_row(vt, L1, 2 * w + 1, L3, 2 * k2 + 1);
+          }
         } else {
-          memcpy(&pub_next[(size_t)S * w], &L1.obs[(size_t)S * k1], sizeof(float) * S);
-          memcpy(&pub_next[(size_t)S * (W + 2 * w)], &L2.obs[(size_t)S * 2 * k1], sizeof(float) * 2 * S);
+          vt.copy_row(e, w, L1.env, k1);
+          if (on) {
+            copy_level_row(vt, tmp, 2 * w, L2, 2 * k1);
+            copy_level_row(vt, tmp, 2 * w + 1, L2, 2 * k1 + 1);
+          }
         }
       }
-      t0_next = Clock::now();
-      tag_next = jh_persist_publish(c->persist, 3 * W, pub_next.data());
+      if (!two && on)
+        for (int i = 2 * w0; i < 2 * w1; ++i) copy_level_row(vt, L1, i, tmp, i);
+      const auto t2 = Clock::now();
+      if (dbg) d_book += secs(q3, t2);
+      c->t_env += secs(t1, t2);
+      t0[h] = t0_next;
+      std::swap(pub[h], pub_next[h]);
+      if (on) {
+        rc = speculate(h, t_next);
+        if (rc) return env_failed(c, rc);
+      }
     }
-    const auto q3 = dbg ? Clock::now() : t1;
-    if (dbg) d_publish += secs(t1, q3);
-    for (int w = 0; w < W; ++w) {
-      capture_row(c, r, w, t, hz.data() + (size_t)w * no);
-      if (two) capture_row(c, r, w, t + 1, hz2.data() + (size_t)w * no);
-    }
-    count_act(c, r, t, secs(t0, t1));
-    if (extra) {
-      t = t_next;
-      break;
-    }
-    if (!two) { tmp.env = L3.env; tmp.init(2 * W, S); }
-    for (int w = 0; w < W; ++w) {
-      const int k1 = 2 * w + (int)a0[w];
-      store_row(c, r, w, t, &pub[(size_t)S * w], &L1.next[(size_t)S * k1], &a0[w], L1.rw[k1], L1.dn[k1]);
-      if (two) {
-        const int k2 = 2 * k1 + (int)a1[w];
-        store_row(c, r, w, t + 1, &L1.obs[(size_t)S * k1], &L2.next[(size_t)S * k2], &a1[w], L2.rw[k2], L2.dn[k2]);
-        vt.copy_row(e, w, L2.env, k2);
-        if (t_next < steps) {
-          copy_level_row(vt, L1, 2 * w, L3, 2 * k2);
-          copy_level_row(vt, L1, 2 * w + 1, L3, 2 * k2 + 1);
-        }
-      } else {
-        vt.copy_row(e, w, L1.env, k1);
-        copy_level_row(vt, tmp, 2 * w, L2, 2 * k1);
-        copy_level_row(vt, tmp, 2 * w + 1, L2, 2 * k1 + 1);
-      }
-    }
-    if (!two)
-      for (int i = 0; i < 2 * W; ++i) copy_level_row(vt, L1, i, tmp, i);
-    c->steps += two ? 2 : 1;
-    const auto t2 = Clock::now();
-    if (dbg) d_book += secs(q3, t2);
-    c->t_env += secs(t1, t2);
+    ctr += extra ? 0 : two ? 2 : 1;
+    c->net->act_ctr = ctr;
+    c->steps += extra ? 0 : two ? 2 : 1;
     t = t_next;
-    tag = tag_next;
-    t0 = t0_next;
-    pub.swap(pub_next);
+    ++k;
+    if (dead) break;
   }
   *t_done = t;
   if (dbg && n_ex > 0 && (c->runs % 16) == 15)
-    fprintf(stderr, "[jh_collect] host us per exchange (%d exchanges): fork %.2f  wait %.2f  sample %.2f  publish %.2f  book %.2f\n", n_ex, d_fork / n_ex * 1e6,
-            d_wait / n_ex * 1e6, d_sample / n_ex * 1e6, d_publish / n_ex * 1e6, d_book / n_ex * 1e6);
-  if (c->dbg_persist && (c->runs % 16) == 15) jh_persist_dump_debug(c->persist, collector_steps(c, T));
+    fprintf(stderr, "[jh_collect] host us per %s (%d of them): fork %.2f  wait %.2f  sample %.2f  publish %.2f  book %.2f\n", NP == 2 ? "half-exchange" : "exchange", n_ex,
+            d_fork / n_ex * 1e6, d_wait / n_ex * 1e6, d_sample / n_ex * 1e6, d_publish / n_ex * 1e6, d_book / n_ex * 1e6);
+  if (c->dbg_persist && (c->runs % 16) == 15 && !dead) jh_persist_dump_debug(c->persist, collector_steps(c, T));
   return JH_OK;
 }
 
diff --git a/jorldy_amd/csrc/jh_persist.hip b/jorldy_amd/csrc/jh_persist.hip
--- a/jorldy_amd/csrc/jh_persist.hip
+++ b/jorldy_amd/csrc/jh_persist.hip
@@ -22,6 +22,7 @@
   unsigned long long* mbox;
   float4* dpart;
   int split;
+  int rows_rt[2];
 };
 
 __device__ __forceinline__ void persist_poll_issue(const void* gsrc, unsigned lds_off) {
@@ -80,8 +81,9 @@
   for (int i = threadIdx.x; i < D * 128 * PI; i += 256) (&s_ring[0][0])[i] = 0ull;
   __syncthreads();
 
+  const int rows_mine = p.rows_rt[rt];
   const int g0 = p.split ? rt * 16 * S : 0;
-  const int n_gran = p.split ? (p.W - 16 * rt < 16 ? p.W - 16 * rt : 16) * S : p.W * S;
+  const int n_gran = p.split ? rows_mine * S : p.W * S;
   const int n16 = (n_gran + 1) >> 1;
   const char* my_src = reinterpret_cast<const char*>(p.obs_gran + g0) + 16 * (lane < n16 ? lane : 0);
   const bool poller = !p.mbox || (p.split ? tile == 0 : blockIdx.x == 0);
@@ -239,7 +241,7 @@
       __builtin_amdgcn_wave_barrier();
       __builtin_amdgcn_fence(__ATOMIC_RELEASE, "workgroup");
       const int g = lane >> 4, row = lane & 15;
-      if (g < p.G && 16 * rt + row < p.W) {
+      if (g < p.G && row < rows_mine) {
         const f32x4 gq = (f32x4){s_out[row][3 * g], s_out[row][3 * g + 1], s_out[row][3 * g + 2], __uint_as_float(tag)};
         if (p.dpart) {
           float4* dst = p.dpart + ((size_t)(rt * p.G + g) * 16 + row) * tiles_n + tile;
@@ -252,7 +254,7 @@
     }
     if (p.dpart && tile == 0) {
       const int g = lane >> 4, row = lane & 15;
-      const bool mine = g < p.G && 16 * rt + row < p.W;
+      const bool mine = g < p.G && row < rows_mine;
       const int per = tiles_n / 4;
       bool ok = true;
       if (mine) {
@@ -378,11 +380,17 @@
   else JH_LAUNCH_NAMED("jh_act_persist_kernel", (jh_act_persist_kernel<SP, NCH, 1, 1>), dim3(grid), dim3(256), 0, st, a);
 }
 
-int jh_persist_begin(jh_persist* p, int W, int T, hipStream_t st, int split) {
+static int persist_poll_instructions(int granules) { return ((granules + 1) / 2 + 63) / 64; }
+bool jh_persist_can_split(const jh_persist* p, int rows0, int rows1) {
+  const int S = p->net->S;
+  return rows0 >= 1 && rows0 <= 16 && rows1 >= 1 && rows1 <= 16 && persist_poll_instructions(rows0 * S) == persist_poll_instructions(rows1 * S);
+}
+int jh_persist_begin(jh_persist* p, int W, int T, hipStream_t st, const int* half_rows) {
   jh_pponet* n = p->net;
-  JH_ARG(W > 0 && W <= 32 && W * n->S <= kPersistMaxGranules && T > 0 && (!split || W == 32));
-  const int win = split ? 16 * n->S : W * n->S;
-  const int pi = ((win + 1) / 2 + 63) / 64;
+  const bool split = half_rows != nullptr;
+  JH_ARG(T > 0 && (split ? jh_persist_can_split(p, half_rows[0], half_rows[1]) && W == half_rows[0] + half_rows[1] : W > 0 && W <= 32 && W * n->S <= kPersistMaxGranules));
+  const int win = split ? half_rows[0] * n->S : W * n->S;
+  const int pi = persist_poll_instructions(win);
   PersistArgs a{};
   a.W = W; a.S = n->S; a.H = n->H; a.T = T; a.G = p->G;
   a.W1 = n->params + n->o_w1; a.b1 = n->params + n->o_b1; a.W2 = n->params + n->o_w2; a.b2 = n->params + n->o_b2;
@@ -400,16 +408,18 @@
   a.period = depth > 1 ? period : 0;
   static const int relay = getenv("JH_PERSIST_RELAY") ? atoi(getenv("JH_PERSIST_RELAY")) : 1;
   a.mbox = relay ? p->mbox : nullptr;
-  const int reduce = getenv("JH_PERSIST_REDUCE") ? atoi(getenv("JH_PERSIST_REDUCE")) : (split ? 1 : 0);
+  const int reduce = getenv("JH_PERSIST_REDUCE") ? atoi(getenv("JH_PERSIST_REDUCE")) : (split && W == 32 ? 1 : 0);
   p->reduced = reduce == 1;
   a.dpart = p->reduced ? p->dpart : nullptr;
   a.split = split ? 1 : 0;
-  p->split = split != 0;
+  p->split = split;
   a.max_polls = 600000;
   p->flag_h[0] = 0;
   const int nch = n->H / 64;
   const int sp = (n->S + 3) / 4 * 4;
-  const int rt = W > 16 ? 2 : 1;
+  const int rt = split || W > 16 ? 2 : 1;
+  a.rows_rt[0] = split ? half_rows[0] : (W < 16 ? W : 16);
+  a.rows_rt[1] = split ? half_rows[1] : (W > 16 ? W - 16 : 0);
   p->rows_ld = 16 * rt;
   a.rows_ld = p->rows_ld;
   const int grid = p->tiles * rt;
@@ -439,23 +449,25 @@
 }
 
 unsigned jh_persist_seq(const jh_persist* p) { return p->seq; }
-void jh_persist_publish_rows(jh_persist* p, int r0, int r1, const float* h_obs, unsigned tag) {
+void jh_persist_publish_rows(jh_persist* p, int row0, int n, const float* h_obs, unsigned tag) {
   const int S = p->net->S;
-  if (r1 > p->rows_published) p->rows_published = r1;
-  for (int i = r0 * S; i < r1 * S; ++i) {
+  unsigned long long* dst = p->gran_h + (size_t)row0 * S;
+  for (int i = 0; i < n * S; ++i) {
     unsigned bits;
     memcpy(&bits, h_obs + i, 4);
-    __atomic_store_n(p->gran_h + i, ((unsigned long long)tag << 32) | bits, __ATOMIC_RELEASE);
+    __atomic_store_n(dst + i, ((unsigned long long)tag << 32) | bits, __ATOMIC_RELEASE);
   }
   if ((int)(tag - p->seq) > 0) p->seq = tag;
 }
 
-static int persist_collect(jh_persist* p, const int* rows, int n_rows, unsigned tag, float* h_heads, int r_first, bool block_order);
+static int persist_collect(jh_persist* p, const int* rows, int n_rows, unsigned tag, float* h_heads, int r_first, bool block_order, int pf_rows);
 int jh_persist_collect_rows(jh_persist* p, const int* rows, int n_rows, unsigned tag, float* h_heads) {
-  return persist_collect(p, rows, n_rows, tag, h_heads, 0, !rows && n_rows > 16);
-}
-int jh_persist_collect_range(jh_persist* p, int r0, int n_rows, unsigned tag, float* h_heads) { return persist_collect(p, nullptr, n_rows, tag, h_heads, r0, true); }
-static int persist_collect(jh_persist* p, const int* rows, int n_rows, unsigned tag, float* h_heads, int r_first, bool block_order) {
+  return persist_collect(p, rows, n_rows, tag, h_heads, 0, !rows && n_rows > 16, (!rows && p->rows_published > n_rows) ? p->rows_published - n_rows : 0);
+}
+int jh_persist_collect_range(jh_persist* p, int r0, int n_rows, unsigned tag, float* h_heads, int pf_rows) {
+  return persist_collect(p, nullptr, n_rows, tag, h_heads, r0, n_rows == 16 && pf_rows == 0, pf_rows);
+}
+static int persist_collect(jh_persist* p, const int* rows, int n_rows, unsigned tag, float* h_heads, int r_first, bool block_order, int pf_rows) {
   const int n_out = p->n_out, G = p->G, ld = p->rows_ld, tiles = p->reduced ? 1 : p->tiles;
   volatile unsigned* abort_w = p->flag_h;
   struct alignas(16) Gran16 { unsigned w[4]; };
@@ -496,12 +508,11 @@
     return JH_OK;
   }
   int missing = n_rows;
-  const int pf_rows = (!rows && p->rows_published > n_rows) ? p->rows_published - n_rows : 0;
   for (int k = 0; k < n_rows; ++k) have[k] = 0;
   for (long spin = 0; spin < 40000000L && missing; ++spin) {
     for (int k = 0; k < n_rows; ++k) {
       if (have[k]) continue;
-      const int wq = rows ? rows[k] : k;
+      const int wq = rows ? rows[k] : r_first + k;
       float acc[12] = {0, 0, 0, 0, 0, 0, 0, 0, 0, 0, 0, 0};
       bool ok = true;
       for (int t = 0; t < tiles && ok; ++t)
@@ -510,8 +521,8 @@
           if (__atomic_load_n(reinterpret_cast<const unsigned*>(gp) + 3, __ATOMIC_ACQUIRE) != tag) { ok = false; break; }
 #if defined(__x86_64__)
           if (pf_rows > 0 && k == 0) {
-            const char* q = reinterpret_cast<const char*>(part + ((size_t)t * G + g) * ld + n_rows);
-            for (int b = 0; b < pf_rows * 16; b += 64) _mm_prefetch(q + b, _MM_HINT_T0);
+            const char* q = reinterpret_cast<const char*>(part + ((size_t)t * G + g) * ld + r_first + n_rows);
+            for (int b = -(int)(reinterpret_cast<uintptr_t>(q) & 63); b < pf_rows * 16; b += 64) _mm_prefetch(q + b, _MM_HINT_T0);
           }
 #endif
           alignas(16) unsigned w4[4];
```

Result: faster. 1.316 million, median of 6 (+7.9%).
